# jyegerlehner/tensorflow-wavenet

Hardware: AMD Instinct MI355X
Metric: audio samples/sec (train, default wavenet_params.json) (higher is better)
Workload: dtype f32

## Files before the change

include/wavenet_hip.h:

```cpp
#ifndef WAVENET_HIP_H_
#define WAVENET_HIP_H_

#include <stdint.h>

#ifdef __cplusplus
extern "C" {
#endif

#define WN_OK 0
#define WN_ERR_BAD_SHAPE (-1)
#define WN_ERR_UNSUPPORTED (-2)
#define WN_ERR_MISALIGNED (-3)
#define WN_ERR_LAUNCH (-4)
#define WN_ERR_NULL (-5)

int wn_version(void);
const char* wn_error_string(int code);

int wn_mu_law_thresholds_host(int Q, float* thr_out);
int wn_mu_law_decode_table_host(int Q, float* lut_out);
int wn_mu_law_encode(const float* audio, int32_t* codes, long n,
                     const float* thr_dev, int Q, void* stream);
int wn_mu_law_decode(const int32_t* codes, float* audio, long n,
                     const float* lut_dev, int Q, void* stream);
// ... 55 lines not shown

int wn_layer_bwd2_slabs(int B, int T);
int wn_layer_bwd2_wimg_floats(void);
int wn_layer_bwd2_pack(const float* layer0, long layer_stride, float* wimg,
                       int L, void* stream);
int wn_layer_bwd2(const float* x, const float* z, const float* sg,
                  const float* dZ, const float* dxin, float* dx_out,
                  const float* wblock, const float* wimg, float* slabs,
                  float* tile_colsum, int B, int T, int dilation,
                  void* stream);

#define WN_STACK_VARIANT(rows, waves) (((rows) & 0x3f) | (((waves) & 0xf) << 8))
long wn_stack_flag_count(int B, int T, int L);
int wn_stack_tile_rows(int B, int T, int variant);
int wn_stack_wimg_floats(void);
int wn_stack_pack(const float* layer0, long layer_stride, float* wimg_fwd,
                  float* wimg_bwd, int L, void* stream);
int wn_stack_fwd(float* X, float* Z, float* SG, const float* wimg,
                 const float* bias, long bias_layer_stride,
                 int bias_clip_stride, const int* dilations, unsigned* flags,
                 unsigned* ctl, float* poison, int L, int B, int T, int save_sg,
                 int variant, void* stream);
int wn_stack_fwd_skip_ok(int B, int T, int S, int variant);
long wn_stack_skip_img_floats(int L);
int wn_stack_skip_pack(const float* skip_w, int L, float* img, void* stream);
int wn_stack_fwd_skip(float* X, float* Z, float* SG, const float* wimg,
                      const float* bias, long bias_layer_stride,
                      int bias_clip_stride, const int* dilations, unsigned* flags,
                      unsigned* ctl, float* poison, int L, int B, int T, int save_sg,
                      int variant, const float* skip_img, const float* skip_bsum,
                      float* h1, void* stream);
int wn_stack_fwd_lc(float* X, float* Z, float* SG, const float* wimg,
                    const float* bias, long bias_layer_stride,
                    int bias_clip_stride, const int* dilations, unsigned* flags,
                    unsigned* ctl, float* poison, int L, int B, int T, int save_sg,
                    int variant, const float* lc_add, long lc_row_stride,
                    void* stream);
int wn_stack_bwd_slabs(int B, int T, int variant);
int wn_stack_fwd_waves(int B, int T, int variant);
int wn_stack_bwd_waves(int B, int T, int variant, int* tiles_per_wave);
int wn_stack_bwd(const float* X, const float* Z, const float* SG,
                 const float* dZ, float* DX, long dx_layer_stride, float* Q,
                 const float* wimg, float* slabs,
                 long slab_layer_stride, float* tilesum, const int* dilations,
                 unsigned* flags, unsigned* ctl, float* poison, int L, int B,
                 int T, int variant, void* stream);
int wn_stack_bwd_lc(const float* X, const float* Z, const float* SG,
                    const float* dZ, float* DX, long dx_layer_stride, float* Q,
                    const float* wimg, float* slabs,
                    long slab_layer_stride, float* tilesum, const int* dilations,
                    unsigned* flags, unsigned* ctl, float* poison, int L, int B,
                    int T, int variant, float* lc_da, long lc_row_stride,
                    void* stream);

int wn_gemm_nn(const float* A, long lda, int a_planes, long a_plane_stride,
               const float* W, int ldw, const float* bias, const float* mask,
               long ld_mask, const float* addend, long ld_add, float* C,
               long ldc, int c_planes, long c_plane_stride, float* Cpre,
               long M, int N, int K, int relu, void* stream);

long wn_gemm_split_w_bytes(int K, int N);
int wn_gemm_nn_split(const float* A, long lda, int a_planes,
                     long a_plane_stride, const float* W, int ldw,
                     const float* bias, const float* mask, long ld_mask,
                     const float* addend, long ld_add, float* C, long ldc,
                     int c_planes, long c_plane_stride, float* Cpre, long M,
                     int N, int K, int relu, void* w_scratch, int nprod,
                     void* stream);
long wn_gemm_tn_slab_floats(int Mw, int Nw);
int wn_gemm_tn_tail_rows(int Mw, int Nw);
int wn_gemm_tn_splits(long rows, int Mw, int Nw, int kind);
int wn_gemm_tn_split(const float* A, long lda, int a_planes,
                     long a_plane_stride, const float* G, long ldg,
                     float* slabs, int splits, long rows, int Mw, int Nw,
                     int want_colsum, int nprod, void* stream);
int wn_gemm_tn(const float* A, long lda, int a_planes, long a_plane_stride,
               const int32_t* codes, int shift, int T, const float* G,
               long ldg, float* slabs, int splits, long rows, int Mw, int Nw,
               int want_colsum, void* stream);
int wn_reduce_slabs(const float* slabs, int num_slabs, long slab_stride,
                    int batch, long in_batch_stride, long offset, long n,
                    float* dst, long out_batch_stride, int replicate,
                    long rep_stride, void* stream);
int wn_reduce_slabs_mt(const float* slabs, int num_slabs, long slab_stride,
                       long n_main, float* dst_main, long n_tail, float* dst_tail,
                       int replicate, long rep_stride, int tail_rows, void* stream);
int wn_reduce_pair_slabs(const float* slabs, int num_slabs, int CB, int K,
                         int has_dense, int use_bias, float* layer_grad, int C,
                         long off_bias, int tap0, int Ktot, void* stream);
int wn_transpose(const float* in, int rows, int cols, long in_ld, float* out,
                 long out_ld, void* stream);

int wn_xent_partials(long rows);
int wn_xent(const float* logits, long ld, const int32_t* q, float* dlogits,
            float* loss_partials, int B, int T, int Q, int tf_quirk,
            void* stream);
int wn_xent_masked(const float* logits, long ld, const int32_t* q,
                   const int32_t* lengths, const float* inv_den,
                   float* dlogits, float* loss_partials, int B, int T, int Q,
                   int tf_quirk, void* stream);
int wn_xent_window(const float* logits, long ld, const int32_t* q,
                   const int32_t* starts, const int32_t* lengths,
                   const float* inv_den, float* dlogits, float* loss_partials,
                   int B, int T, int Q, int tf_quirk, void* stream);
long wn_xent_score_scratch_floats(long rows);
int wn_xent_score(const float* logits, long ld, const int32_t* q,
                  const int32_t* lengths, float* row_nll, double* clip_nll,
                  int32_t* clip_count, int32_t* clip_correct, float* scratch,
                  int B, int T, int Q, void* stream);
int wn_xent_score_window(const float* logits, long ld, const int32_t* q,
                         const int32_t* starts, const int32_t* lengths,
                         float* row_nll, double* clip_nll, int32_t* clip_count,
                         int32_t* clip_correct, float* scratch, int B, int T,
                         int Q, void* stream);
int wn_softmax64_row(const float* logits_row, int Q, float* proba,
                     void* stream);

int wn_adam(float* p, const float* g, float* m, float* v, long n, float lr_t,
            float beta1, float beta2, float eps, float grad_scale, float l2,
            const float* l2_mask, void* stream);
int wn_momentum(float* p, const float* g, float* acc, long n, float lr,
                float momentum, float grad_scale, float l2,
                const float* l2_mask, void* stream);
int wn_rmsprop(float* p, const float* g, float* ms, float* mom, long n,
               float lr, float decay, float momentum, float eps,
               float grad_scale, float l2, const float* l2_mask,
               void* stream);
int wn_grad_norm_partials_count(void);
int wn_grad_norm_partials(const float* g, long n, double* partials,
                          void* stream);
int wn_adam_clip(float* p, const float* g, float* m, float* v, long n,
                 float lr_t, float beta1, float beta2, float eps,
                 float grad_scale, float l2, const float* l2_mask,
                 const double* partials, int nparts, float clip_norm,
                 float* ema, float ema_decay, float* norm_out, void* stream);
int wn_momentum_clip(float* p, const float* g, float* acc, long n, float lr,
                     float momentum, float grad_scale, float l2,
                     const float* l2_mask, const double* partials, int nparts,
                     float clip_norm, float* ema, float ema_decay,
                     float* norm_out, void* stream);
int wn_rmsprop_clip(float* p, const float* g, float* ms, float* mom, long n,
                    float lr, float decay, float momentum, float eps,
                    float grad_scale, float l2, const float* l2_mask,
                    const double* partials, int nparts, float clip_norm,
                    float* ema, float ema_decay, float* norm_out,
                    void* stream);
int wn_l2_partials_count(void);
int wn_l2_partials(const float* p, long n, const float* mask, float* partials,
                   void* stream);

int wn_gc_bias(const float* layer0, long layer_stride, long off_bias,
               long off_gc, int G, const float* emb, int card,
               const int32_t* ids, float* out, int L, int B, int ch,
               void* stream);
int wn_colsum_clip_chunks(int T);
int wn_colsum_clip(const float* plane0, const float* plane1, int B, int T,
                   float* part, float* out, void* stream);
int wn_gc_grad(const float* layer0, long layer_stride, long off_gc, int G,
               const float* emb, int card, const int32_t* ids,
               const float* dsum, int L, int B, float* glayer0, float* gemb,
               float* scratch , int ch, void* stream);

int wn_causal_conv(const float* x, const float* w, float* y, int B, int T,
                   int Cin, int Cout, int K, int dilation, void* stream);
int wn_time_to_batch(const float* in, float* out, int B, int T, int C,
                     int dilation, void* stream);
int wn_batch_to_time(const float* in, float* out, int B_out, int U, int C,
                     int dilation, void* stream);

int wn_diag_mfma_peak(float* out, int blocks, int iters, void* stream);

int wn_axpy(float* y, const float* x, float a, const float* mask, long n,
            void* stream);
int wn_fill(float* p, long n, float value, void* stream);
int wn_sum_rows(const float* in, int rows, int n, float* out, void* stream);

long wn_fastgen_state_floats(const int32_t* dilations_host, int L);
int wn_fastgen_init(float* state, long state_floats, int32_t* cursors, int L,
                    void* stream);
int wn_fastgen_run(const float* params_causal, const float* layer0,
                   long layer_stride, const float* skip_w,
                   const float* skip_bsum, const float* post1_w,
                   const float* post1_b, const float* post2_w,
                   const float* post2_b, const float* gc_bias_fg,
                   const int32_t* dilations_dev, int L, int S, int Q,
                   float* state, int32_t* cursors, int32_t* samples_io,
                   int n_given, int n_steps, float temperature, uint64_t seed,
                   float* proba_out, int proba_every, int use_biases,
                   int push, void* stream);

long wn_fastgen_wide_coop_bytes(int L, int C, int S, int Q);
int wn_fastgen_run_wide(const float* params_causal, const float* layer0,
                        long layer_stride, const float* skip_w,
                        const float* skip_bsum, const float* post1_w,
                        const float* post1_b, const float* post2_w,
                        const float* post2_b, const float* gc_bias_fg,
                        const int32_t* dilations_dev, int L, int C, int S, int Q,
                        float* state, int32_t* cursors, int32_t* samples_io,
                        int n_given, int n_steps, float temperature,
                        uint64_t seed, float* proba_out, int proba_every,
                        int use_biases, int push, void* coop, void* stream);

int wn_fastgen_step(const float* params_causal, const float* layer0,
                    long layer_stride, const float* skip_w,
                    const float* skip_bsum, const float* post1_w,
                    const float* post1_b, const float* post2_w,
                    const float* post2_b, const float* gc_bias_fg,
                    const int32_t* dilations_dev, int L, int S, int Q,
                    float* state, int32_t* cursors, int32_t* samples_io,
                    const int32_t* ctl, float* proba_out, int use_biases,
                    const float* cw_img, float* pre, float* z_all, float* h1,
                    float* h2, float* logits, void* stream);
int wn_fastgen_finish(int Q, int32_t* cursors, int32_t* samples_io,
                      const int32_t* ctl, float* proba_out, const float* logits,
                      void* stream);

int wn_fastgen_persist_workgroups(int L, int S, int Q);
int wn_fastgen_persist_role(int block, int total, int nseg);
long wn_fastgen_persist_ll_words(int L, int S, int Q);
int wn_fastgen_persist(const float* params_causal, const float* layer0,
                       long layer_stride, const float* skip_w,
                       const float* skip_bsum, const float* post1_w,
                       const float* post1_b, const float* post2_w,
                       const float* post2_b, const float* gc_bias_fg,
                       const int32_t* dilations_dev, int L, int S, int Q,
                       float* state, int32_t* cursors, int32_t* samples_io,
                       const int32_t* ctl, float* proba_out, int use_biases,
                       const float* cw_img, float* pre, float* z_all, float* h1,
                       float* h2, float* logits, unsigned* sync,
                       unsigned long long* ll, int n_steps, void* stream);
int wn_fastgen_pre(const float* layer0, long layer_stride,
                   const float* gc_bias_fg, const int32_t* dilations_dev,
                   int L, const float* state, const int32_t* cursors,
                   float* pre, void* stream);
int wn_fastgen_pack(const float* layer0, long layer_stride, float* img, int L,
                    void* stream);

int wn_fastgen_batch_rows(int B);
long wn_fastgen_batch_state_floats(const int32_t* dilations_host, int L, int B);
int wn_fastgen_batch_init(float* state, long state_floats, int32_t* cursors,
                          int32_t* prev, int B, void* stream);
int wn_fastgen_batch_pre(const float* layer0, long layer_stride,
                         const float* gc_bias_fg, int bias_stream_stride,
                         const int32_t* dilations_dev, int L, int B,
                         const float* state, const int32_t* cursors, float* pre,
                         void* stream);
int wn_fastgen_batch_step(const float* params_causal, const float* layer0,
                          long layer_stride, const float* skip_w,
                          const float* skip_bsum, const float* post1_w,
                          const float* post1_b, const float* post2_w,
                          const float* post2_b, const float* gc_bias_fg,
                          int bias_stream_stride, const int32_t* dilations_dev,
                          int L, int S, int Q, int B, float* state,
                          int32_t* cursors, int32_t* prev, int32_t* samples_io,
                          const int32_t* ctl, const uint64_t* seeds,
                          float* proba_out, int use_biases, float* pre,
                          float* z_all, float* h1, float* h2, float* logits,
                          void* stream);
// ... 203 lines not shown
```

tensorflow-wavenet_amd/csrc/wn_gemm.hip:

```cpp
#include "wn_common.h"
#include <cstdlib>
#include <cstddef>
#include <cstring>

struct GemmNN {
  const float* A;
  long lda;
  long a_plane_stride;
  int a_planes;
  const float* W;
  int ldw;
  const float* bias;
  const float* mask;
  long ld_mask;
  const float* addend;
  long ld_add;
  float* C;
  long ldc;
  long c_plane_stride;
  int c_planes;
  float* Cpre;
  long M;
  int N, K;
  int relu;
  int tiles_n;
  int nwg;
  int tiles_m;
  int tile_rows;
};

typedef const __attribute__((address_space(1))) void* gptr_t;
typedef __attribute__((address_space(3))) void* lptr_t;

#define NN_TM 128
#define NN_TN 128
#define NN_KC 32
#ifndef NN3_PF
#define NN3_PF 2
#endif

__device__ __forceinline__ int xcd_remap(int bid, int nwg) {
  const int q = nwg >> 3, r = nwg & 7, xcd = bid & 7, idx = bid >> 3;
  const int base = xcd < r ? xcd * (q + 1) : r * (q + 1) + (xcd - r) * q;
  return base + idx;
}

#define EP_LD 68
#ifndef EP_ST_AUX
#define EP_ST_AUX 2
#endif
#ifndef EP_LD_AUX
#define EP_LD_AUX 2
#endif
typedef unsigned ep_u32x4 __attribute__((ext_vector_type(4)));
__device__ __forceinline__ __amdgpu_buffer_rsrc_t ep_rsrc(const float* base) {
  return __builtin_amdgcn_make_buffer_rsrc((void*)base, 0, 0x7fffffff, 0x00020000);
}
__device__ __forceinline__ void gemm_epilogue(const GemmNN& g, f32x16 (&acc)[2][2],
                                              float* lds, long m0, int n0,
                                              int wm, int wn, int wave, int lane,
                                              long m_end = -1) {
  if (m_end < 0) m_end = g.M;
  const int j = lane & 31, h = lane >> 5;
  float* tile = lds + wave * (32 * EP_LD);
  const int rr = lane >> 4, cc = (lane & 15) * 4;
  const int nw = n0 + wn * 64;
  const bool ncol = nw + cc < g.N;
  f32x4 bias4 = {0.f, 0.f, 0.f, 0.f};
  if (g.bias && ncol) bias4 = *reinterpret_cast<const f32x4*>(g.bias + nw + cc);
  const int vC = g.c_planes ? (int)(((long)(cc >> 5) * g.c_plane_stride + rr * 32 + (cc & 31)) * 4)
                            : (int)((rr * g.ldc + cc) * 4);
  const int sC = g.c_planes ? 4 * 32 * 4 : (int)(4 * g.ldc * 4);
  const int vP = (int)((rr * g.ldc + cc) * 4);
  const int sP = (int)(4 * g.ldc * 4);
  const int vM = (int)((rr * g.ld_mask + cc) * 4), sM = (int)(4 * g.ld_mask * 4);
  const bool addp = g.addend && g.c_planes && g.ld_add == 0;
  const int vA = addp ? vC : (int)((rr * g.ld_add + cc) * 4);
  const int sA = addp ? sC : (int)(4 * g.ld_add * 4);
#pragma unroll
  for (int fm = 0; fm < 2; ++fm) {
    __builtin_amdgcn_wave_barrier();
#pragma unroll
    for (int fn = 0; fn < 2; ++fn)
// ... 1087 lines not shown

  const int prow = lane >> 5, pcol = (lane & 31) * 4;
  int am = m0 + pcol;
  am = am < g.Mw ? am : g.Mw - 4;
  int gn = n0 + pcol;
  gn = gn < g.Nw ? gn : g.Nw - 4;
  auto stage = [&](int c, int st) {
    float* base = smem + st * STAGE;
    const long r0 = r_begin + (long)c * KR;
#pragma unroll
    for (int q = 0; q < 2; ++q) {
      const int p = wave + 4 * q;
      const long row = r0 + 2 * p + prow;
      const float* src = g.a_planes
                             ? g.A + (long)(am >> 5) * g.a_plane_stride + row * 32 + (am & 31)
                             : g.A + row * g.lda + am;
      __builtin_amdgcn_global_load_lds((gptr_t)src, (lptr_t)(base + p * 256), 16, 0, 0);
      __builtin_amdgcn_global_load_lds((gptr_t)(g.G + row * g.ldg + gn),
                                       (lptr_t)(base + KR * TT + p * 256), 16, 0, 0);
    }
  };

  f32x16 acc[2][2];
#pragma unroll
  for (int a = 0; a < 2; ++a)
#pragma unroll
    for (int b = 0; b < 2; ++b) acc[a][b] = frag_zero();
  float cs[2] = {0.f, 0.f};

  if (nchunks > 0) stage(0, 0);
  for (int c = 0; c < nchunks; ++c) {
    const int st = c & 1;
    asm volatile("s_waitcnt vmcnt(0)\n\ts_barrier" ::: "memory");
    if (c + 1 < nchunks) stage(c + 1, st ^ 1);
    const float* al = smem + st * STAGE + 8 * h * TT + wm * 64 + i;
    const float* gl = smem + st * STAGE + KR * TT + 8 * h * TT + wn * 64 + i;
    Split3 as[2], gs[2];
#pragma unroll
    for (int f = 0; f < 2; ++f) {
      float v[8];
#pragma unroll
      for (int e = 0; e < 8; ++e) v[e] = al[e * TT + f * 32];
      as[f] = split3(v);
    }
#pragma unroll
    for (int f = 0; f < 2; ++f) {
      float v[8];
#pragma unroll
      for (int e = 0; e < 8; ++e) {
        v[e] = gl[e * TT + f * 32];
        cs[f] += v[e];
      }
      gs[f] = split3(v);
    }
#pragma unroll
    for (int a = 0; a < 2; ++a)
#pragma unroll
      for (int b = 0; b < 2; ++b) mma_split<NPROD>(acc[a][b], as[a], gs[b]);
  }

  float* slab = g.slabs + (long)split * g.slab_stride;
#pragma unroll
  for (int a = 0; a < 2; ++a)
#pragma unroll
    for (int b = 0; b < 2; ++b) {
      const int n = n0 + wn * 64 + b * 32 + i;
      if (n >= g.Nw) continue;
#pragma unroll
      for (int rr = 0; rr < 16; ++rr) {
        const int m = m0 + wm * 64 + a * 32 + 8 * (rr >> 2) + 4 * h + (rr & 3);
        if (m < g.Mw) slab[(long)m * g.Nw + n] = acc[a][b][rr];
      }
    }
  if (g.want_colsum && tm == 0 && wm == 0) {
#pragma unroll
    for (int b = 0; b < 2; ++b) {
      const float v = cs[b] + __shfl_xor(cs[b], 32);
      const int n = n0 + wn * 64 + b * 32 + i;
      if (h == 0 && n < g.Nw) slab[(long)g.Mw * g.Nw + n] = v;
    }
  }
}

__global__ void reduce_slabs_kernel(const float* __restrict__ slabs,
                                    int num_slabs, long slab_stride,
                                    long in_batch_stride, long offset, long n,
                                    float* __restrict__ dst,
                                    long out_batch_stride, int replicate,
                                    long rep_stride) {
  const long e = (long)blockIdx.x * blockDim.x + threadIdx.x;
  if (e >= n) return;
  const int b = blockIdx.y;
  const float* p = slabs + (long)b * in_batch_stride + offset + e;
  float s0 = 0.f, s1 = 0.f, s2 = 0.f, s3 = 0.f;
  int s = 0;
  for (; s + 3 < num_slabs; s += 4) {
    s0 += p[(long)s * slab_stride];
    s1 += p[(long)(s + 1) * slab_stride];
    s2 += p[(long)(s + 2) * slab_stride];
    s3 += p[(long)(s + 3) * slab_stride];
  }
  for (; s < num_slabs; ++s) s0 += p[(long)s * slab_stride];
  const float v = (s0 + s1) + (s2 + s3);
  for (int r = 0; r < replicate; ++r)
    dst[(long)b * out_batch_stride + (long)r * rep_stride + e] = v;
}

template <int PARTS>
__global__ void reduce_slabs4_kernel(const float* __restrict__ slabs,
                                     int num_slabs, long slab_stride,
                                     long in_batch_stride, long offset, long n4,
                                     float* __restrict__ dst,
                                     long out_batch_stride, int replicate,
                                     long rep_stride) {
  __shared__ f32x4 part[PARTS > 1 ? PARTS : 1][64];
  const int col = threadIdx.x & 63, pt = threadIdx.x >> 6;
  const long e = (long)blockIdx.x * 64 + col;
  const int b = blockIdx.y;
  const int per = (num_slabs + PARTS - 1) / PARTS;
  const int s0 = pt * per, s1 = min(num_slabs, s0 + per);
  f32x4 acc[8];
#pragma unroll
  for (int k = 0; k < 8; ++k) acc[k] = f32x4{0.f, 0.f, 0.f, 0.f};
  if (e < n4) {
    const f32x4* p = reinterpret_cast<const f32x4*>(slabs + (long)b * in_batch_stride + offset) + e;
    const long st = slab_stride / 4;
    int s = s0;
    for (; s + 7 < s1; s += 8) {
      f32x4 v[8];
#pragma unroll
      for (int k = 0; k < 8; ++k) v[k] = p[(long)(s + k) * st];
#pragma unroll
      for (int k = 0; k < 8; ++k) acc[k] += v[k];
    }
#pragma unroll
    for (int k = 0; k < 7; ++k)
      if (s + k < s1) acc[k] += p[(long)(s + k) * st];
  }
  f32x4 v = ((acc[0] + acc[1]) + (acc[2] + acc[3])) + ((acc[4] + acc[5]) + (acc[6] + acc[7]));
  if (PARTS > 1) {
    part[pt][col] = v;
    __syncthreads();
    if (pt != 0) return;
    if (PARTS == 4) v = (part[0][col] + part[1][col]) + (part[2][col] + part[3][col]);
    else v = part[0][col] + part[1][col];
  }
  if (e >= n4) return;
  for (int r = 0; r < replicate; ++r)
    *reinterpret_cast<f32x4*>(dst + (long)b * out_batch_stride + (long)r * rep_stride + 4 * e) = v;
}

#ifndef RMT_PARTS
#define RMT_PARTS 4
#endif
__global__ __launch_bounds__(64 * RMT_PARTS) void reduce_slabs_mt_kernel(
    const float* __restrict__ slabs, int num_slabs, long slab_stride, long n_main4,
    float* __restrict__ dst_main, long n_tail4, float* __restrict__ dst_tail,
    int replicate, long rep_stride, int tail_rows) {
  __shared__ f32x4 part[RMT_PARTS][64];
  const int col = threadIdx.x & 63, pt = threadIdx.x >> 6;
  const long e = (long)blockIdx.x * 64 + col;
  const long n4 = n_main4 + n_tail4;
  const int per = (num_slabs + RMT_PARTS - 1) / RMT_PARTS;
  const int s0 = min(num_slabs, pt * per), s1 = min(num_slabs, s0 + per);
  f32x4 acc[8];
#pragma unroll
  for (int k = 0; k < 8; ++k) acc[k] = f32x4{0.f, 0.f, 0.f, 0.f};
  if (e < n4) {
    const f32x4* p = reinterpret_cast<const f32x4*>(slabs) + e;
    const long st = slab_stride / 4;
    int s = s0;
    for (; s + 7 < s1; s += 8) {
      f32x4 v[8];
#pragma unroll
      for (int k = 0; k < 8; ++k) v[k] = p[(long)(s + k) * st];
#pragma unroll
      for (int k = 0; k < 8; ++k) acc[k] += v[k];
    }
#pragma unroll
    for (int k = 0; k < 7; ++k)
      if (s + k < s1) acc[k] += p[(long)(s + k) * st];
    if (e >= n_main4 && tail_rows > 1) {
      const int nv = (s1 - s0) * (tail_rows - 1);
      int v = 0;
      for (; v + 7 < nv; v += 8) {
        f32x4 w[8];
#pragma unroll
        for (int k = 0; k < 8; ++k) {
          const int q = s0 + (v + k) / (tail_rows - 1), t = 1 + (v + k) % (tail_rows - 1);
          w[k] = p[(long)q * st + (long)t * n_tail4];
        }
#pragma unroll
        for (int k = 0; k < 8; ++k) acc[k] += w[k];
      }
      for (; v < nv; ++v) {
        const int q = s0 + v / (tail_rows - 1), t = 1 + v % (tail_rows - 1);
        acc[v & 7] += p[(long)q * st + (long)t * n_tail4];
      }
    }
  }
  part[pt][col] = ((acc[0] + acc[1]) + (acc[2] + acc[3])) + ((acc[4] + acc[5]) + (acc[6] + acc[7]));
  __syncthreads();
  if (pt != 0 || e >= n4) return;
  f32x4 v = f32x4{0.f, 0.f, 0.f, 0.f};
#pragma unroll
  for (int q = 0; q < RMT_PARTS; q += 4)
    v += (part[q][col] + part[q + 1][col]) + (part[q + 2][col] + part[q + 3][col]);
  if (e < n_main4) {
    reinterpret_cast<f32x4*>(dst_main)[e] = v;
  } else {
    for (int r = 0; r < replicate; ++r)
      *reinterpret_cast<f32x4*>(dst_tail + (long)r * rep_stride + 4 * (e - n_main4)) = v;
  }
}

#define RPS_PARTS 16
__global__ __launch_bounds__(64 * RPS_PARTS) void reduce_pair_slabs_kernel(
    const float* __restrict__ slabs, int num_slabs, int CB, int K, int has_dense,
    int use_bias, float* __restrict__ g, int C, long off_bias, int tap0, int Ktot) {
  __shared__ f32x4 part[RPS_PARTS][64];
  const int WF = (2 * K + 1) * 1024, n4 = (WF + 96) / 4;
  const int col = threadIdx.x & 63, pt = threadIdx.x >> 6;
  const int e4 = blockIdx.x * 64 + col;
  const int pair = blockIdx.y, a = pair / CB, b = pair - a * CB;
  const int per = (num_slabs + RPS_PARTS - 1) / RPS_PARTS;
  const int s0 = min(num_slabs, pt * per), s1 = min(num_slabs, s0 + per);
  f32x4 acc[8];
#pragma unroll
  for (int k = 0; k < 8; ++k) acc[k] = f32x4{0.f, 0.f, 0.f, 0.f};
  if (e4 < n4) {
    const f32x4* p = reinterpret_cast<const f32x4*>(
                         slabs + (size_t)pair * num_slabs * (WF + 96)) + e4;
    const long st = (WF + 96) / 4;
    int s = s0;
    for (; s + 7 < s1; s += 8) {
      f32x4 v[8];
#pragma unroll
      for (int k = 0; k < 8; ++k) v[k] = p[(long)(s + k) * st];
#pragma unroll
      for (int k = 0; k < 8; ++k) acc[k] += v[k];
    }
#pragma unroll
    for (int k = 0; k < 7; ++k)
      if (s + k < s1) acc[k] += p[(long)(s + k) * st];
  }
  part[pt][col] = ((acc[0] + acc[1]) + (acc[2] + acc[3])) + ((acc[4] + acc[5]) + (acc[6] + acc[7]));
  __syncthreads();
  if (pt != 0 || e4 >= n4) return;
  f32x4 v = f32x4{0.f, 0.f, 0.f, 0.f};
#pragma unroll
  for (int q = 0; q < RPS_PARTS; q += 4)
    v += (part[q][col] + part[q + 1][col]) + (part[q + 2][col] + part[q + 3][col]);
  const int e = 4 * e4;
  if (e < WF) {
    const int m = e >> 10, r = (e >> 5) & 31, c = e & 31;
    if (m == 2 * K && !has_dense) return;
    const int md = m < K ? tap0 + m : m < 2 * K ? Ktot + tap0 + (m - K) : 2 * Ktot;
    *reinterpret_cast<f32x4*>(g + ((size_t)md * C + a * 32 + r) * C + b * 32 + c) = v;
  } else if (a == 0 && use_bias) {
    const int q = (e - WF) >> 5, c = (e - WF) & 31;
    if (q == 2 && !has_dense) return;
    *reinterpret_cast<f32x4*>(g + off_bias + (size_t)q * C + b * 32 + c) = v;
  }
}

__global__ void transpose_pad_kernel(const float* __restrict__ in, int rows,
                                     int cols, long in_ld,
                                     float* __restrict__ out, long out_ld) {
  __shared__ float tile[32][33];
  const int bx = blockIdx.x * 32, by = blockIdx.y * 32;
  const int tx = threadIdx.x & 31, ty = threadIdx.x >> 5;
  for (int k = ty; k < 32; k += 8) {
    const int r = by + k, c = bx + tx;
    tile[k][tx] = (r < rows && c < cols) ? in[(long)r * in_ld + c] : 0.f;
  }
  __syncthreads();
  for (int k = ty; k < 32; k += 8) {
    const int c = bx + k, r = by + tx;
    if (c < cols && r < rows) out[(long)c * out_ld + r] = tile[tx][k];
  }
}

template <int MODE>
__global__ __launch_bounds__(256) void mfma_peak_kernel(float* out, int iters) {
  __shared__ float lds[4096];
  for (int k = threadIdx.x; k < 4096; k += 256) lds[k] = 1.0f + k * 1e-4f;
  __syncthreads();
  f32x16 a0 = frag_zero(), a1 = frag_zero(), a2 = frag_zero(), a3 = frag_zero();
  float x = 1.0f + threadIdx.x * 1e-3f, y = 0.5f - threadIdx.x * 1e-3f;
  const float* lp = lds + (threadIdx.x & 63);
  for (int it = 0; it < iters; ++it) {
#pragma unroll
    for (int u = 0; u < 8; ++u) {
      if (MODE == 1) {
        x = lp[(u * 128 + it) & 4095 & ~63];
        y = lp[((u * 128 + 64 + it) & 4095) & ~63];
      }
      a0 = __builtin_amdgcn_mfma_f32_32x32x2f32(x, y, a0, 0, 0, 0);
      a1 = __builtin_amdgcn_mfma_f32_32x32x2f32(y, x, a1, 0, 0, 0);
      a2 = __builtin_amdgcn_mfma_f32_32x32x2f32(x, x, a2, 0, 0, 0);
      a3 = __builtin_amdgcn_mfma_f32_32x32x2f32(y, y, a3, 0, 0, 0);
    }
  }
  float s = 0.f;
#pragma unroll
  for (int r = 0; r < 16; ++r) s += a0[r] + a1[r] + a2[r] + a3[r];
  out[blockIdx.x * 256 + threadIdx.x] = s;
}

extern "C" {

int wn_diag_mfma_peak(float* out, int blocks, int iters, void* stream) {
  if (!out) return WN_ERR_NULL;
  if (blocks <= 0 || iters == 0) return WN_ERR_BAD_SHAPE;
  if (iters > 0)
    hipLaunchKernelGGL(mfma_peak_kernel<0>, dim3(blocks), dim3(256), 0,
                       (hipStream_t)stream, out, iters);
  else
    hipLaunchKernelGGL(mfma_peak_kernel<1>, dim3(blocks), dim3(256), 0,
                       (hipStream_t)stream, out, -iters);
  return wn_check_launch();
}

static int gemm_nn_describe(GemmNN& g, const float* A, long lda, int a_planes,
               long a_plane_stride, const float* W, int ldw, const float* bias,
               const float* mask, long ld_mask, const float* addend, long ld_add,
               float* C, long ldc, int c_planes, long c_plane_stride, float* Cpre,
               long M, int N, int K, int relu) {
  if (!A || !W || !C) return WN_ERR_NULL;
  if (M <= 0 || N <= 0 || K <= 0) return WN_ERR_BAD_SHAPE;
  if ((N & 3) || (K & 3) || (ldw & 3)) return WN_ERR_UNSUPPORTED;
  if (a_planes) {
    if (K != a_planes * 32) return WN_ERR_BAD_SHAPE;
  } else if (lda & 3) {
    return WN_ERR_UNSUPPORTED;
  }
  if (c_planes) {
    if (N != c_planes * 32) return WN_ERR_BAD_SHAPE;
  } else if (ldc & 3) {
    return WN_ERR_UNSUPPORTED;
  }
  if ((mask && (ld_mask & 3)) || (addend && (ld_add & 3)))
    return WN_ERR_UNSUPPORTED;
  if (addend && ld_add == 0 && !c_planes) return WN_ERR_BAD_SHAPE;
  if (c_planes && c_plane_stride * 4 >= (1L << 31)) return WN_ERR_UNSUPPORTED;
  const void* ptrs[] = {A, W, bias, mask, addend, C, Cpre};
  for (const void* p : ptrs)
    if (p && !wn_aligned16(p)) return WN_ERR_MISALIGNED;
  g.A = A; g.lda = lda; g.a_plane_stride = a_plane_stride; g.a_planes = a_planes;
  g.W = W; g.ldw = ldw; g.bias = bias; g.mask = mask; g.ld_mask = ld_mask;
  g.addend = addend; g.ld_add = ld_add; g.C = C; g.ldc = ldc;
  g.c_plane_stride = c_plane_stride; g.c_planes = c_planes; g.Cpre = Cpre;
  g.M = M; g.N = N; g.K = K; g.relu = relu;
  long tiles_m = (M + NN_TM - 1) / NN_TM;
  g.tiles_n = (N + NN_TN - 1) / NN_TN;
  g.tile_rows = NN_TM;
  const long nwg = tiles_m * g.tiles_n;
  if (nwg > 0x7fffffffL) return WN_ERR_BAD_SHAPE;
  g.nwg = (int)nwg;
  g.tiles_m = (int)tiles_m;
  return WN_OK;
}

// ... 135 lines not shown
  g.tiles_m = (Mw + 127) / 128;
  g.tiles_n = (Nw + 127) / 128;
  dim3 grid(g.tiles_m * g.tiles_n, splits), block(256);
  hipStream_t s = (hipStream_t)stream;
  if (nprod == 3) hipLaunchKernelGGL(gemm_tn_split_kernel<3>, grid, block, 0, s, g);
  else if (nprod == 9) hipLaunchKernelGGL(gemm_tn_split_kernel<9>, grid, block, 0, s, g);
  else hipLaunchKernelGGL(gemm_tn_split_kernel<6>, grid, block, 0, s, g);
  return wn_check_launch();
}

int wn_gemm_tn(const float* A, long lda, int a_planes, long a_plane_stride,
               const int32_t* codes, int shift, int T, const float* G,
               long ldg, float* slabs, int splits, long rows, int Mw, int Nw,
               int want_colsum, void* stream) {
  if (!G || !slabs) return WN_ERR_NULL;
  if (!A && !codes) return WN_ERR_NULL;
  if (rows <= 0 || Mw <= 0 || Nw <= 0 || splits <= 0) return WN_ERR_BAD_SHAPE;
  if (a_planes && Mw != a_planes * 32) return WN_ERR_BAD_SHAPE;
  if (codes && T <= 0) return WN_ERR_BAD_SHAPE;
  GemmTN g;
  g.A = A; g.lda = lda; g.a_plane_stride = a_plane_stride; g.a_planes = a_planes;
  g.codes = codes; g.shift = shift; g.T = T > 0 ? T : 1; g.G = G; g.ldg = ldg;
  g.slabs = slabs; g.slab_stride = wn_gemm_tn_slab_floats(Mw, Nw);
  g.rows = rows;
  long rps = (rows + splits - 1) / splits;
  rps = (rps + 95) / 96 * 96;
  g.rows_per_split = rps;
  g.Mw = Mw; g.Nw = Nw; g.want_colsum = want_colsum;
  hipStream_t s = (hipStream_t)stream;
  if (!codes && (lda % 4 == 0) && (ldg % 4 == 0) && wn_aligned16(A) &&
      wn_aligned16(G)) {
    int mf2 = 0, nf2 = 0;
    tn_wg_tile(Mw, Nw, &mf2, &nf2);
    if (mf2 && nf2) {
      g.tiles_m = Mw / (mf2 * 32);
      g.tiles_n = Nw / (4 * nf2 * 32);
      dim3 grid2(g.tiles_m * g.tiles_n, splits), block2(256);
      const long rps = (rows + splits - 1) / splits + 96;
      const long a_bytes = (a_planes ? 5 * a_plane_stride + rps * 32 : rps * lda) * 4;
      const bool dma = a_bytes < (1L << 31) && rps * ldg * 4 < (1L << 31);
#define LAUNCH2(mf, nf)                                                          \
  do {                                                                           \
    if (dma) hipLaunchKernelGGL((gemm_tn3_kernel<mf, nf>), grid2, block2, 0, s, g); \
    else hipLaunchKernelGGL((gemm_tn2_kernel<mf, nf>), grid2, block2, 0, s, g);  \
  } while (0)
      if (mf2 == 5 && nf2 == 2) LAUNCH2(5, 2);
      else if (mf2 == 5) LAUNCH2(5, 1);
      else if (nf2 == 2) LAUNCH2(4, 2);
      else LAUNCH2(4, 1);
#undef LAUNCH2
      return wn_check_launch();
    }
  }
  if (want_colsum == 2) return WN_ERR_UNSUPPORTED;
  const int m32 = (Mw + 31) / 32, n32 = (Nw + 31) / 32;
  int NF = (n32 % 2 == 0) ? 2 : 1;
  int MF;
  if (codes) { NF = 1; MF = (m32 % 2 == 0) ? 2 : 1; }
  else if (m32 % 5 == 0) MF = 5;
  else if (m32 % 4 == 0) MF = 4;
  else if (m32 % 2 == 0) MF = 2;
  else MF = 1;
  g.tiles_m = (m32 + MF - 1) / MF;
  g.tiles_n = (n32 + NF - 1) / NF;
  const int wtiles = g.tiles_m * g.tiles_n;
  dim3 grid((wtiles + 3) / 4, splits), block(256);
#define LAUNCH(mf, nf) \
  hipLaunchKernelGGL((gemm_tn_kernel<mf, nf>), grid, block, 0, s, g)
  if (NF == 2) {
    if (MF == 5) LAUNCH(5, 2);
    else if (MF == 4) LAUNCH(4, 2);
    else if (MF == 2) LAUNCH(2, 2);
    else LAUNCH(1, 2);
  } else {
    if (MF == 5) LAUNCH(5, 1);
    else if (MF == 4) LAUNCH(4, 1);
    else if (MF == 2) LAUNCH(2, 1);
    else LAUNCH(1, 1);
  }
#undef LAUNCH
  return wn_check_launch();
}

__global__ __launch_bounds__(64) void reduce_slabs_wave_kernel(
    const float* __restrict__ slabs, int num_slabs, long slab_stride,
    long in_batch_stride, long offset, float* __restrict__ dst,
    long out_batch_stride, int replicate, long rep_stride) {
  const long e = blockIdx.x;
  const int b = blockIdx.y;
  const float* p = slabs + (long)b * in_batch_stride + offset + e;
  float v = 0.f;
  for (int s = threadIdx.x; s < num_slabs; s += 64) v += p[(long)s * slab_stride];
#pragma unroll
  for (int o = 32; o >= 1; o >>= 1) v += __shfl_xor(v, o);
  if (threadIdx.x == 0)
    for (int r = 0; r < replicate; ++r)
      dst[(long)b * out_batch_stride + (long)r * rep_stride + e] = v;
}

int wn_reduce_slabs(const float* slabs, int num_slabs, long slab_stride,
                    int batch, long in_batch_stride, long offset, long n,
                    float* dst, long out_batch_stride, int replicate,
                    long rep_stride, void* stream) {
  if (!slabs || !dst) return WN_ERR_NULL;
  if (num_slabs <= 0 || n <= 0 || batch <= 0 || replicate <= 0)
    return WN_ERR_BAD_SHAPE;
  if (n <= 4 && num_slabs >= 256) {
    hipLaunchKernelGGL(reduce_slabs_wave_kernel, dim3((unsigned)n, batch),
                       dim3(64), 0, (hipStream_t)stream, slabs, num_slabs,
                       slab_stride, in_batch_stride, offset, dst,
                       out_batch_stride, replicate, rep_stride);
    return wn_check_launch();
  }
  if (((n | offset | slab_stride | in_batch_stride | out_batch_stride | rep_stride) & 3) == 0 &&
      wn_aligned16(slabs) && wn_aligned16(dst)) {
    const long n4 = n / 4;
    dim3 grid4((unsigned)((n4 + 63) / 64), batch);
    const bool split = num_slabs >= 32 && (long)grid4.x * batch <= 4096;
    if (split)
      hipLaunchKernelGGL(reduce_slabs4_kernel<4>, grid4, dim3(256), 0, (hipStream_t)stream,
                         slabs, num_slabs, slab_stride, in_batch_stride, offset, n4,
                         dst, out_batch_stride, replicate, rep_stride);
    else
      hipLaunchKernelGGL(reduce_slabs4_kernel<1>, grid4, dim3(64), 0, (hipStream_t)stream,
                         slabs, num_slabs, slab_stride, in_batch_stride, offset, n4,
                         dst, out_batch_stride, replicate, rep_stride);
    return wn_check_launch();
  }
  dim3 grid((unsigned)((n + 255) / 256), batch), block(256);
  hipLaunchKernelGGL(reduce_slabs_kernel, grid, block, 0, (hipStream_t)stream,
                     slabs, num_slabs, slab_stride, in_batch_stride, offset, n,
                     dst, out_batch_stride, replicate, rep_stride);
  return wn_check_launch();
}

int wn_reduce_slabs_mt(const float* slabs, int num_slabs, long slab_stride,
                       long n_main, float* dst_main, long n_tail, float* dst_tail,
                       int replicate, long rep_stride, int tail_rows, void* stream) {
  if (!slabs || !dst_main || (n_tail > 0 && !dst_tail)) return WN_ERR_NULL;
  if (num_slabs <= 0 || n_main <= 0 || n_tail < 0 || replicate < 1 || tail_rows < 1 ||
      slab_stride < n_main + (long)tail_rows * n_tail)
    return WN_ERR_BAD_SHAPE;
  if (((n_main | n_tail | slab_stride | rep_stride) & 3) != 0) return WN_ERR_UNSUPPORTED;
  if (!wn_aligned16(slabs) || !wn_aligned16(dst_main) || (dst_tail && !wn_aligned16(dst_tail)))
    return WN_ERR_MISALIGNED;
  const long n4 = (n_main + n_tail) / 4;
  hipLaunchKernelGGL(reduce_slabs_mt_kernel, dim3((unsigned)((n4 + 63) / 64)), dim3(64 * RMT_PARTS), 0,
                     (hipStream_t)stream, slabs, num_slabs, slab_stride, n_main / 4, dst_main,
                     n_tail / 4, dst_tail, replicate, rep_stride, tail_rows);
  return wn_check_launch();
}

int wn_reduce_pair_slabs(const float* slabs, int num_slabs, int CB, int K,
                         int has_dense, int use_bias, float* layer_grad, int C,
                         long off_bias, int tap0, int Ktot, void* stream) {
  if (!slabs || !layer_grad) return WN_ERR_NULL;
  if (num_slabs <= 0 || CB <= 0 || K < 1 || C != CB * 32 || off_bias < 0 || (off_bias & 3) ||
      tap0 < 0 || Ktot < tap0 + K)
    return WN_ERR_BAD_SHAPE;
  if (!wn_aligned16(slabs) || !wn_aligned16(layer_grad)) return WN_ERR_MISALIGNED;
  const int n4 = ((2 * K + 1) * 1024 + 96) / 4;
  hipLaunchKernelGGL(reduce_pair_slabs_kernel, dim3((n4 + 63) / 64, CB * CB), dim3(64 * RPS_PARTS), 0,
                     (hipStream_t)stream, slabs, num_slabs, CB, K, has_dense, use_bias,
                     layer_grad, C, off_bias, tap0, Ktot);
  return wn_check_launch();
}

int wn_transpose(const float* in, int rows, int cols, long in_ld, float* out,
                 long out_ld, void* stream) {
  if (!in || !out) return WN_ERR_NULL;
  if (rows <= 0 || cols <= 0) return WN_ERR_BAD_SHAPE;
  dim3 grid((cols + 31) / 32, (rows + 31) / 32), block(256);
  hipLaunchKernelGGL(transpose_pad_kernel, grid, block, 0, (hipStream_t)stream,
                     in, rows, cols, in_ld, out, out_ld);
  return wn_check_launch();
}

}
```

tensorflow-wavenet_amd/csrc/wn_misc.hip:

```cpp
#include "wn_common.h"
#include <stdlib.h>
#include <cmath>

#pragma clang fp contract(off)
static inline int mu_chain_host(float x, int Q) {
  const float mu = (float)(Q - 1);
  const float ax = std::fabs(x);
  const float arg = 1.0f + mu * ax;
  const float num = (float)std::log((double)arg);
  const float den = (float)std::log((double)(1.0f + mu));
  const float mag = num / den;
  const float sgn = (x > 0.f) ? 1.f : ((x < 0.f) ? -1.f : 0.f);
  float v = sgn * mag;
  v = v + 1.0f;
  v = v / 2.0f;
  v = v * mu;
  v = v + 0.5f;
  return (int)v;
}

static inline uint32_t f2key(float f) {
  uint32_t u;
  __builtin_memcpy(&u, &f, 4);
  return (u & 0x80000000u) ? ~u : (u | 0x80000000u);
}
static inline float key2f(uint32_t k) {
  uint32_t u = (k & 0x80000000u) ? (k & 0x7FFFFFFFu) : ~k;
  float f;
  __builtin_memcpy(&f, &u, 4);
  return f;
}

__device__ __forceinline__ int mu_chain_dev(float x, int Q) {
  const float mu = (float)(Q - 1);
  const float arg = __fadd_rn(1.0f, __fmul_rn(mu, fabsf(x)));
  const float num = (float)log((double)arg);
  const float den = (float)log((double)__fadd_rn(1.0f, mu));
  const float mag = __fdiv_rn(num, den);
  const float sgn = (x > 0.f) ? 1.f : ((x < 0.f) ? -1.f : 0.f);
  float v = __fmul_rn(sgn, mag);
  v = __fadd_rn(v, 1.0f);
  v = __fdiv_rn(v, 2.0f);
  v = __fmul_rn(v, mu);
  v = __fadd_rn(v, 0.5f);
  return (int)v;
}

__global__ void mu_law_encode_kernel(const float* __restrict__ audio,
                                     int32_t* __restrict__ codes, long n,
                                     const float* __restrict__ thr, int Q) {
  extern __shared__ float sthr[];
  for (int i = threadIdx.x; i < Q - 1; i += blockDim.x) sthr[i] = thr[i];
  __syncthreads();
  for (long idx = (long)blockIdx.x * blockDim.x + threadIdx.x; idx < n;
       idx += (long)gridDim.x * blockDim.x) {
    const float x = audio[idx];
    int code;
    if (x >= -1.f && x <= 1.f) {
      int lo = 0, hi = Q - 1;
      while (lo < hi) {
        const int mid = (lo + hi) >> 1;
        if (sthr[mid] <= x) lo = mid + 1; else hi = mid;
      }
      code = lo;
    } else {
      code = mu_chain_dev(x, Q);
    }
    codes[idx] = code;
  }
}

__device__ __forceinline__ float mu_decode_dev(int code, int Q) {
  const float mu = (float)(Q - 1);
  const float s = __fsub_rn(__fmul_rn(2.0f, __fdiv_rn((float)code, mu)), 1.0f);
  const float p = (float)pow((double)__fadd_rn(1.0f, mu), (double)fabsf(s));
  const float mag = __fmul_rn(__fdiv_rn(1.0f, mu), __fsub_rn(p, 1.0f));
  const float sgn = (s > 0.f) ? 1.f : ((s < 0.f) ? -1.f : 0.f);
  return __fmul_rn(sgn, mag);
}

__global__ void mu_law_decode_kernel(const int32_t* __restrict__ codes,
                                     float* __restrict__ audio, long n,
                                     const float* __restrict__ lut, int Q) {
  for (long idx = (long)blockIdx.x * blockDim.x + threadIdx.x; idx < n;
       idx += (long)gridDim.x * blockDim.x) {
    const int c = codes[idx];
    audio[idx] = (c >= 0 && c < Q) ? lut[c] : mu_decode_dev(c, Q);
  }
}

__global__ void causal_gather_kernel(const int32_t* __restrict__ q,
                                     const float* __restrict__ Wc,
                                     float* __restrict__ x0, long rows, int T,
                                     int Q, int K, int ldw) {
  const long idx = (long)blockIdx.x * blockDim.x + threadIdx.x;
  const long row = idx >> 3;
  const int c4 = (idx & 7) * 4;
  if (row >= rows) return;
  const int t = (int)(row % T);
  f32x4 v = {0.f, 0.f, 0.f, 0.f};
  const int extra = (K - 1) / 2;
  for (int k = 0; k < K; ++k) {
    const int s = (K - 1 - k) + extra;
    if (t < s) continue;
    const int code = q[row - s];
    if (code >= 0 && code < Q)
      v += *reinterpret_cast<const f32x4*>(Wc + ((long)k * Q + code) * ldw + c4);
  }
  *reinterpret_cast<f32x4*>(x0 + row * 32 + c4) = v;
}

__global__ void scalar_causal_fwd_kernel(const float* __restrict__ audio,
                                         const float* __restrict__ W,
                                         float* __restrict__ x0, long rows,
                                         int T, int K0, int ldw) {
  const long idx = (long)blockIdx.x * blockDim.x + threadIdx.x;
  const long row = idx >> 3;
  const int c4 = (idx & 7) * 4;
  if (row >= rows) return;
  const int t = (int)(row % T);
  f32x4 v = {0.f, 0.f, 0.f, 0.f};
  const int extra = (K0 - 1) / 2;
  for (int k = 0; k < K0; ++k) {
    const int s = (K0 - 1 - k) + extra;
    if (t - s < 0) continue;
    const float a = audio[row - s];
    const f32x4 w = *reinterpret_cast<const f32x4*>(W + (long)k * ldw + c4);
    v += a * w;
  }
  *reinterpret_cast<f32x4*>(x0 + row * 32 + c4) = v;
}

__global__ __launch_bounds__(1024) void scalar_causal_wgrad_kernel(
    const float* __restrict__ audio, const float* __restrict__ dx0,
    float* __restrict__ slabs, long rows, long rows_per_split, int T, int K0) {
  const int c = threadIdx.x & 31;
  const long r0 = (long)blockIdx.x * rows_per_split;
  long r1 = r0 + rows_per_split;
  if (r1 > rows) r1 = rows;
  for (int k = threadIdx.x >> 5; k < K0; k += 32) {
    const int s = (K0 - 1 - k) + (K0 - 1) / 2;
    float acc = 0.f;
    int t = (int)(r0 % T);
    for (long r = r0; r < r1; ++r) {
      if (t >= s) acc = fmaf(audio[r - s], dx0[r * 32 + c], acc);
      if (++t == T) t = 0;
    }
    slabs[(long)blockIdx.x * K0 * 32 + k * 32 + c] = acc;
  }
}

__global__ void gc_bias_kernel(const float* __restrict__ layer0, long layer_stride,
                               long off_bias, long off_gc, int G,
                               const float* __restrict__ emb, int card,
                               const int32_t* __restrict__ ids,
                               float* __restrict__ out, int B, int ch) {
  const int l = blockIdx.x, b = blockIdx.y;
  const float* blk = layer0 + (long)l * layer_stride;
  for (int c = threadIdx.x; c < 2 * ch; c += blockDim.x) {
    float v = blk[off_bias + c];
    if (emb) {
      const int id = ids[b];
      if (id >= 0 && id < card) {
        const float* w = blk + off_gc + (c >= ch ? (long)G * ch : 0) + (c % ch);
        const float* e = emb + (long)id * G;
        for (int g = 0; g < G; ++g) v += e[g] * w[(long)g * ch];
      }
    }
    out[((long)l * B + b) * 2 * ch + c] = v;
  }
}

__global__ __launch_bounds__(256) void colsum_clip_kernel(
    const float* __restrict__ P0, const float* __restrict__ P1, int T,
    int rows_per_chunk, float* __restrict__ part) {
  __shared__ float red[8][64];
  const int b = blockIdx.y, chunk = blockIdx.x;
  const int c = threadIdx.x & 31, w = threadIdx.x >> 5;
  const int t0 = chunk * rows_per_chunk;
  const int t1 = min(T, t0 + rows_per_chunk);
  const float* p0 = P0 + (long)b * T * 32;
  const float* p1 = P1 + (long)b * T * 32;
  float s0 = 0.f, s1 = 0.f;
  for (int t = t0 + w; t < t1; t += 8) {
    s0 += p0[(long)t * 32 + c];
    s1 += p1[(long)t * 32 + c];
  }
  red[w][c] = s0;
  red[w][32 + c] = s1;
  __syncthreads();
  if (threadIdx.x < 64) {
    float v = 0.f;
// ... 43 lines not shown
                                   float* __restrict__ gemb) {
  extern __shared__ float tmp[];
  const int tid = threadIdx.x;
  for (int e = tid; e < card * G; e += blockDim.x) gemb[e] = 0.f;
  for (int e = tid; e < B * G; e += blockDim.x) {
    float s = 0.f;
    for (int l = 0; l < L; ++l) s += part[(long)l * B * G + e];
    tmp[e] = s;
  }
  __syncthreads();
  for (int gi = tid; gi < G; gi += blockDim.x) {
    for (int b = 0; b < B; ++b) {
      const int id = ids[b];
      if (id < 0 || id >= card) continue;
      gemb[(long)id * G + gi] += tmp[b * G + gi];
    }
  }
}

__global__ void causal_conv_kernel(const float* __restrict__ x,
                                   const float* __restrict__ w,
                                   float* __restrict__ y, int B, int T, int Cin,
                                   int Cout, int K, int d) {
  const long idx = (long)blockIdx.x * blockDim.x + threadIdx.x;
  const long total = (long)B * T * Cout;
  if (idx >= total) return;
  const int co = (int)(idx % Cout);
  const long bt = idx / Cout;
  const int t = (int)(bt % T);
  const long b = bt / T;
  float acc = 0.f;
  for (int k = 0; k < K; ++k) {
    const long shift = (long)(K - 1 - k + (K - 1) / 2) * d;
    if (t - shift < 0) continue;
    const float* xr = x + ((b * T) + (t - shift)) * Cin;
    const float* wk = w + (long)k * Cin * Cout + co;
    for (int ci = 0; ci < Cin; ++ci) acc += xr[ci] * wk[(long)ci * Cout];
  }
  y[idx] = acc;
}

__global__ void time_to_batch_kernel(const float* __restrict__ in,
                                     float* __restrict__ out, int B, int T,
                                     int C, int d, int U) {
  const long idx = (long)blockIdx.x * blockDim.x + threadIdx.x;
  const long total = (long)B * d * U * C;
  if (idx >= total) return;
  const int c = (int)(idx % C);
  long r = idx / C;
  const int u = (int)(r % U);
  r /= U;
  const int b = (int)(r % B), p = (int)(r / B);
  const long t = (long)u * d + p;
  out[idx] = t < T ? in[((long)b * T + t) * C + c] : 0.f;
}

__global__ void batch_to_time_kernel(const float* __restrict__ in,
                                     float* __restrict__ out, int B, int U,
                                     int C, int d) {
  const long idx = (long)blockIdx.x * blockDim.x + threadIdx.x;
  const long total = (long)B * d * U * C;
  if (idx >= total) return;
  const int c = (int)(idx % C);
  long r = idx / C;
  const int tt = (int)(r % ((long)U * d));
  const int b = (int)(r / ((long)U * d));
  const int u = tt / d, p = tt % d;
  out[idx] = in[(((long)p * B + b) * U + u) * C + c];
}

__global__ void axpy_kernel(float* __restrict__ y, const float* __restrict__ x,
                            float a, const float* __restrict__ mask, long n) {
  for (long i = (long)blockIdx.x * blockDim.x + threadIdx.x; i < n;
       i += (long)gridDim.x * blockDim.x)
    y[i] += a * x[i] * (mask ? mask[i] : 1.f);
}

__global__ void fill_kernel(float* __restrict__ p, long n, float v) {
  for (long i = (long)blockIdx.x * blockDim.x + threadIdx.x; i < n;
       i += (long)gridDim.x * blockDim.x)
    p[i] = v;
}

__global__ void sum_rows_kernel(const float* __restrict__ in, int rows, int n,
                                float* __restrict__ out) {
  const int c = blockIdx.x * blockDim.x + threadIdx.x;
  if (c >= n) return;
  float s = 0.f;
  int r = 0;
  for (; r + 16 <= rows; r += 16) {
    float v[16];
#pragma unroll
    for (int u = 0; u < 16; ++u) v[u] = in[(long)(r + u) * n + c];
#pragma unroll
    for (int u = 0; u < 16; ++u) s += v[u];
  }
  for (; r < rows; ++r) s += in[(long)r * n + c];
  out[c] = s;
}

extern "C" {

int wn_reduce_slabs(const float* slabs, int num_slabs, long slab_stride,
                    int batch, long in_batch_stride, long offset, long n,
                    float* dst, long out_batch_stride, int replicate,
                    long rep_stride, void* stream);

int wn_version(void) { return 100; }

const char* wn_error_string(int code) {
  switch (code) {
    case WN_OK: return "ok";
    case WN_ERR_BAD_SHAPE: return "bad shape";
    case WN_ERR_UNSUPPORTED: return "unsupported configuration";
    case WN_ERR_MISALIGNED: return "pointer or leading dimension not 16-byte aligned";
    case WN_ERR_LAUNCH: return "kernel launch failed";
    case WN_ERR_NULL: return "null pointer";
    default: return "unknown error";
  }
}

int wn_mu_law_thresholds_host(int Q, float* thr_out) {
  if (!thr_out) return WN_ERR_NULL;
  if (Q < 2) return WN_ERR_BAD_SHAPE;
  const uint32_t lo0 = f2key(-1.0f), hi0 = f2key(1.0f);
  for (int k = 1; k < Q; ++k) {
    uint32_t lo = lo0, hi = hi0;
    if (mu_chain_host(key2f(lo), Q) >= k) { thr_out[k - 1] = key2f(lo); continue; }
    while (hi - lo > 1) {
      const uint32_t mid = lo + (hi - lo) / 2;
      if (mu_chain_host(key2f(mid), Q) >= k) hi = mid; else lo = mid;
    }
    thr_out[k - 1] = key2f(hi);
  }
  return WN_OK;
}

int wn_mu_law_decode_table_host(int Q, float* lut_out) {
  if (!lut_out) return WN_ERR_NULL;
  if (Q < 2) return WN_ERR_BAD_SHAPE;
  const float mu = (float)(Q - 1);
  for (int c = 0; c < Q; ++c) {
    float s = (float)c / mu;
    s = 2.0f * s;
    s = s - 1.0f;
    const float p = (float)std::pow((double)(1.0f + mu), (double)std::fabs(s));
    float mag = 1.0f / mu;
    const float pm1 = p - 1.0f;
    mag = mag * pm1;
    const float sgn = (s > 0.f) ? 1.f : ((s < 0.f) ? -1.f : 0.f);
    lut_out[c] = sgn * mag;
  }
  return WN_OK;
}

int wn_mu_law_encode(const float* audio, int32_t* codes, long n,
                     const float* thr_dev, int Q, void* stream) {
  if (!audio || !codes || !thr_dev) return WN_ERR_NULL;
  if (n <= 0 || Q < 2 || Q > 8192) return WN_ERR_BAD_SHAPE;
  hipLaunchKernelGGL(mu_law_encode_kernel, dim3(grid1d(n, 256)), dim3(256),
                     (Q - 1) * sizeof(float), (hipStream_t)stream, audio, codes,
                     n, thr_dev, Q);
  return wn_check_launch();
}

int wn_mu_law_decode(const int32_t* codes, float* audio, long n,
                     const float* lut_dev, int Q, void* stream) {
  if (!audio || !codes || !lut_dev) return WN_ERR_NULL;
  if (n <= 0 || Q < 2) return WN_ERR_BAD_SHAPE;
  hipLaunchKernelGGL(mu_law_decode_kernel, dim3(grid1d(n, 256)), dim3(256), 0,
                     (hipStream_t)stream, codes, audio, n, lut_dev, Q);
  return wn_check_launch();
}

int wn_causal_gather(const int32_t* q, const float* Wc, float* x0, int B,
                     int T, int Q, int K, int ldw, void* stream) {
  if (!q || !Wc || !x0) return WN_ERR_NULL;
  if (B <= 0 || T <= 0 || Q <= 0 || K <= 0 || ldw < 32 || (ldw & 3))
    return WN_ERR_BAD_SHAPE;
  if (!wn_aligned16(Wc) || !wn_aligned16(x0)) return WN_ERR_MISALIGNED;
  const long rows = (long)B * T;
// ... 180 lines not shown
                     plane0, plane1, T, rpc, part);
  return wn_reduce_slabs(part, chunks, 64, B, (long)chunks * 64, 0, 64, out, 64,
                         1, 0, stream);
}

int wn_gc_grad(const float* layer0, long layer_stride, long off_gc, int G,
               const float* emb, int card, const int32_t* ids,
               const float* dsum, int L, int B, float* glayer0, float* gemb,
               float* scratch, int ch, void* stream) {
  if (!layer0 || !emb || !ids || !dsum || !glayer0 || !gemb || !scratch)
    return WN_ERR_NULL;
  if (L <= 0 || B <= 0 || G <= 0 || card <= 0 || ch < 32) return WN_ERR_BAD_SHAPE;
  if ((size_t)B * G * sizeof(float) > 48 * 1024) return WN_ERR_UNSUPPORTED;
  hipStream_t s = (hipStream_t)stream;
  hipLaunchKernelGGL(gc_grad_kernel, dim3(2 * L), dim3(256), 0, s, layer0,
                     layer_stride, off_gc, G, emb, card, ids, dsum, L, B,
                     glayer0, scratch, ch);
  hipLaunchKernelGGL(gc_grad_emb_kernel, dim3(1), dim3(256),
                     (size_t)B * G * sizeof(float), s, scratch, L, B, G, card,
                     ids, gemb);
  return wn_check_launch();
}

int wn_causal_conv(const float* x, const float* w, float* y, int B, int T,
                   int Cin, int Cout, int K, int dilation, void* stream) {
  if (!x || !w || !y) return WN_ERR_NULL;
  if (B <= 0 || T <= 0 || Cin <= 0 || Cout <= 0 || K <= 0 || dilation <= 0)
    return WN_ERR_BAD_SHAPE;
  const long total = (long)B * T * Cout;
  hipLaunchKernelGGL(causal_conv_kernel, dim3((unsigned)((total + 255) / 256)),
                     dim3(256), 0, (hipStream_t)stream, x, w, y, B, T, Cin,
                     Cout, K, dilation);
  return wn_check_launch();
}

int wn_time_to_batch(const float* in, float* out, int B, int T, int C,
                     int dilation, void* stream) {
  if (!in || !out) return WN_ERR_NULL;
  if (B <= 0 || T <= 0 || C <= 0 || dilation <= 0) return WN_ERR_BAD_SHAPE;
  const int U = (T + dilation - 1) / dilation;
  const long total = (long)B * dilation * U * C;
  hipLaunchKernelGGL(time_to_batch_kernel, dim3((unsigned)((total + 255) / 256)),
                     dim3(256), 0, (hipStream_t)stream, in, out, B, T, C,
                     dilation, U);
  return wn_check_launch();
}

int wn_batch_to_time(const float* in, float* out, int B_out, int U, int C,
                     int dilation, void* stream) {
  if (!in || !out) return WN_ERR_NULL;
  if (B_out <= 0 || U <= 0 || C <= 0 || dilation <= 0) return WN_ERR_BAD_SHAPE;
  const long total = (long)B_out * dilation * U * C;
  hipLaunchKernelGGL(batch_to_time_kernel, dim3((unsigned)((total + 255) / 256)),
                     dim3(256), 0, (hipStream_t)stream, in, out, B_out, U, C,
                     dilation);
  return wn_check_launch();
}

int wn_axpy(float* y, const float* x, float a, const float* mask, long n,
            void* stream) {
  if (!y || !x) return WN_ERR_NULL;
  if (n <= 0) return WN_ERR_BAD_SHAPE;
  hipLaunchKernelGGL(axpy_kernel, dim3(grid1d(n, 256)), dim3(256), 0,
                     (hipStream_t)stream, y, x, a, mask, n);
  return wn_check_launch();
}

int wn_fill(float* p, long n, float value, void* stream) {
  if (!p) return WN_ERR_NULL;
  if (n <= 0) return WN_ERR_BAD_SHAPE;
  hipLaunchKernelGGL(fill_kernel, dim3(grid1d(n, 256)), dim3(256), 0,
                     (hipStream_t)stream, p, n, value);
  return wn_check_launch();
}

int wn_sum_rows(const float* in, int rows, int n, float* out, void* stream) {
  if (!in || !out) return WN_ERR_NULL;
  if (rows <= 0 || n <= 0) return WN_ERR_BAD_SHAPE;
  hipLaunchKernelGGL(sum_rows_kernel, dim3((n + 255) / 256), dim3(256), 0,
                     (hipStream_t)stream, in, rows, n, out);
  return wn_check_launch();
}

}
```

tensorflow-wavenet_amd/csrc/wn_stack.hip:

```cpp
#include "wn_common.h"

#define WN_WAIT_VM0() asm volatile("s_waitcnt vmcnt(0)" ::: "memory")
#define WN_WAIT_LGKM0() asm volatile("s_waitcnt lgkmcnt(0)" ::: "memory")

#define STACK_MAXL 256
#define SF_LD 36
#define SF_MT (32 * SF_LD)
#define SF_OFF_BD (5 * SF_MT)
#define STACK_WBUF 5888

struct StackFwd {
  float* X;
  float* Z;
  float* SG;
  const float* wimg;
  const float* bias;
  long bias_layer_stride;
  int bias_clip_stride;
  const int* dil;
  unsigned* flags;
  unsigned* ctl;
  float* poison;
  int L, B, T;
  long plane;
  const float* skimg;
  const float* sk_bsum;
  float* sk_out;
#ifdef STACK_STAMPS
  unsigned long long* dbg;
#endif
};

#define SK_S 512
#define SK_NT 8
#define SK_WAVE (SK_NT * 2 * 256)
#define SK_AHEAD 3
#define SK_ZB 4

typedef unsigned u32x4 __attribute__((ext_vector_type(4)));

__device__ __forceinline__ RowRegs rows_load_dev(const float* tile0, int lane,
                                                 int lo, int hi) {
  RowRegs R;
  __amdgpu_buffer_rsrc_t rs = __builtin_amdgcn_make_buffer_rsrc(
      (void*)tile0, 0, 0x7fffffff, 0x00020000);
  const int vo = ((lane >> 3) * 32 + (lane & 7) * 4) * 4;
#pragma unroll
  for (int c = 0; c < 4; ++c) {
    const int r = 8 * c + (lane >> 3);
    f32x4 v = {0.f, 0.f, 0.f, 0.f};
    if (r >= lo && r < hi)
      v = __builtin_bit_cast(
          f32x4, __builtin_amdgcn_raw_buffer_load_b128(rs, vo + c * 1024, 0, 16));
    R.v[c] = v;
  }
  return R;
}

template <int AUX>
__device__ __forceinline__ void rows_store_aux(float* tile0, int lane, int hi,
                                               const RowRegs& R) {
  __amdgpu_buffer_rsrc_t rs = __builtin_amdgcn_make_buffer_rsrc(
      (void*)tile0, 0, 0x7fffffff, 0x00020000);
  const int vo = ((lane >> 3) * 32 + (lane & 7) * 4) * 4;
#pragma unroll
  for (int c = 0; c < 4; ++c) {
    const int r = 8 * c + (lane >> 3);
    if (r < hi)
      __builtin_amdgcn_raw_buffer_store_b128(__builtin_bit_cast(u32x4, R.v[c]),
                                             rs, vo + c * 1024, 0, AUX);
  }
}
__device__ __forceinline__ void rows_store_dev(float* tile0, int lane, int hi,
                                               const RowRegs& R) {
  rows_store_aux<16>(tile0, lane, hi, R);
}

__device__ __forceinline__ void wait_flags(const unsigned* fl, int idx,
                                           unsigned epoch, unsigned* ctl,
                                           float* poison, bool& dead, int lane) {
  if (dead) return;
  unsigned spins = 0;
  unsigned long long t_start = 0;
  for (;;) {
    bool pending = false;
    if (idx >= 0)
      pending = __hip_atomic_load(fl + idx, __ATOMIC_RELAXED,
                                  __HIP_MEMORY_SCOPE_AGENT) != epoch;
    if (__builtin_amdgcn_ballot_w64(pending) == 0) break;
    if ((++spins & 63u) == 0) {
      const unsigned long long now = __builtin_amdgcn_s_memrealtime();
      if (t_start == 0) t_start = now;
      if (now - t_start > 200000000ull) {
        if (lane == 0) {
          __hip_atomic_store(ctl + 3, 1u, __ATOMIC_RELAXED, __HIP_MEMORY_SCOPE_AGENT);
          if (poison) *poison = __builtin_nanf("");
        }
        dead = true;
        break;
      }
    }
    __builtin_amdgcn_s_sleep(1);
  }
  asm volatile("" ::: "memory");
}

__device__ __forceinline__ void mma32t_chain(f32x16& acc, const f32x16& frag,
                                             const float* wt_lane, f32x4& pre,
                                             const float* wt_next) {
  f32x4 nxt = pre;
#pragma unroll
  for (int q = 0; q < 4; ++q) {
    const f32x4 a4 = nxt;
    nxt = *reinterpret_cast<const f32x4*>(q < 3 ? wt_lane + 8 * (q + 1) : wt_next);
    __builtin_amdgcn_sched_barrier(0);
#pragma unroll
    for (int e = 0; e < 4; ++e)
      acc = __builtin_amdgcn_mfma_f32_32x32x2f32(a4[e], frag[4 * q + e], acc, 0, 0, 0);
    __builtin_amdgcn_sched_barrier(0);
  }
  pre = nxt;
}

__global__ void stack_pack_kernel(const float* __restrict__ layer0,
                                  long layer_stride, float* __restrict__ img_f,
                                  float* __restrict__ img_b) {
  const bool bwd = blockIdx.y == 1;
  float* img = bwd ? img_b : img_f;
  if (!img) return;
  const float* blk = layer0 + (long)blockIdx.x * layer_stride;
  float* out = img + (size_t)blockIdx.x * STACK_WBUF;
  for (int i = threadIdx.x; i < STACK_WBUF; i += blockDim.x) out[i] = 0.f;
  __syncthreads();
  for (int i = threadIdx.x; i < LAYER_W_FLOATS; i += blockDim.x) {
    const int m = i >> 10, cin = (i >> 5) & 31, cout = i & 31;
    out[bwd ? m * 1024 + cin * 32 + ((((cout >> 2) ^ ((cin >> 1) & 7)) << 2) | (cout & 3))
            : m * SF_MT + cout * SF_LD + cin] = blk[i];
  }
  if (!bwd && threadIdx.x < 32)
    out[SF_OFF_BD + threadIdx.x] = blk[LAYER_OFF_BD + threadIdx.x];
}

__device__ __forceinline__ void wait_lds(const int* p, bool& dead, unsigned* ctl,
                                         float* poison, int lane) {
  unsigned spins = 0;
  while (!dead && __hip_atomic_load(p, __ATOMIC_RELAXED, __HIP_MEMORY_SCOPE_WORKGROUP) == 0) {
    __builtin_amdgcn_s_sleep(1);
    if (++spins > (1u << 24)) {
      dead = true;
      if (lane == 0) {
        __hip_atomic_store(ctl + 3, 1u, __ATOMIC_RELAXED, __HIP_MEMORY_SCOPE_AGENT);
        if (poison) *poison = __builtin_nanf("");
      }
    }
  }
  asm volatile("" ::: "memory");
}

__global__ void stack_skip_pack_kernel(const float* __restrict__ skip_w, float* __restrict__ img) {
  const int l = blockIdx.x >> 2, j = blockIdx.x & 3;
  float* out = img + (size_t)blockIdx.x * SK_WAVE;
  for (int i = threadIdx.x; i < SK_WAVE; i += blockDim.x) {
    const int e = i & 3, lane = (i >> 2) & 63, half = (i >> 8) & 1, nt = i >> 9;
    const int jr = lane & 15, g = lane >> 4;
    out[i] = skip_w[((size_t)l * 32 + 16 * half + 4 * g + e) * SK_S + 128 * j + 16 * nt + jr];
  }
}

struct StackLc {
  float* p;
  long row_stride;
};
__device__ __forceinline__ StackLc stack_lc_arg(StackLc lc) { return lc; }

template <int SAVE, int WAVES, typename... Lc>
__global__ __launch_bounds__(WAVES * 64) void stack_fwd_kernel(StackFwd a, Lc... lc_) {
  constexpr bool LC = sizeof...(Lc) > 0;
  __shared__ __attribute__((aligned(1024))) float wl[2 * STACK_WBUF];
  __shared__ __attribute__((aligned(16))) float tiles[WAVES * 1024];
  __shared__ int s_group;
  __shared__ int s_done[STACK_MAXL], s_ready[STACK_MAXL];
  const int tid = threadIdx.x;
  const int lane = tid & 63;
  const int wave = __builtin_amdgcn_readfirstlane(tid >> 6);
  const int j = lane & 31, h = lane >> 5;
  const int T = a.T, L = a.L;
  const int tiles_per_clip = (T + 31) >> 5;
  const int ntiles = tiles_per_clip * a.B;
  const int ngroups = (ntiles + WAVES - 1) / WAVES;
  const unsigned epoch =
      __hip_atomic_load(a.ctl + 2, __ATOMIC_RELAXED, __HIP_MEMORY_SCOPE_AGENT);
  float* ta = tiles + wave * 1024;
  bool dead = false;
#ifdef STACK_STAMPS
#define SSTAMP(l, i)                                                         \
  if (lane == 0)                                                             \
    a.dbg[(((size_t)blockIdx.x * 16 + wave) * L + (l)) * 12 + (i)] =         \
        __builtin_amdgcn_s_memtime()
  unsigned long long* cal = a.dbg + (size_t)gridDim.x * 16 * L * 12 + (size_t)blockIdx.x * 4;
  if (tid == 0) { cal[0] = __builtin_amdgcn_s_memrealtime(); cal[1] = __builtin_amdgcn_s_memtime(); }
#else
#define SSTAMP(l, i)
#endif

  auto issue_weights = [&](int l, int p0, int step) {
    const float* wb = a.wimg + (size_t)l * STACK_WBUF;
    float* dst = wl + (l & 1) * STACK_WBUF;
    for (int p = p0; p < STACK_WBUF / 256; p += step)
      __builtin_amdgcn_global_load_lds((wn_gptr_t)(wb + p * 256 + lane * 4),
                                       (wn_lptr_t)(dst + p * 256), 16, 0, 0);
  };

  for (;;) {
    if (tid == 0) s_group = (int)atomicAdd(a.ctl, 1u);
    __syncthreads();
    const int g = __builtin_amdgcn_readfirstlane(s_group);
    __syncthreads();
    if (g >= ngroups) break;
    const int tile = g * WAVES + wave;
    const int nactive = min(WAVES, ntiles - g * WAVES);
    const bool any = tile < ntiles;
    const int b = any ? tile / tiles_per_clip : 0;
    const int tt = any ? tile - b * tiles_per_clip : 0;
// ... 1894 lines not shown
```

tensorflow-wavenet_amd/wavenet/_lib.py:

```python
import ctypes
import os

_HERE = os.path.dirname(os.path.abspath(__file__))
LIB_PATH = os.environ.get('WN_LIB_PATH') or os.path.join(
    os.path.dirname(_HERE), 'libwavenet_hip.so')

c_int, c_long, c_float = ctypes.c_int, ctypes.c_long, ctypes.c_float
c_void_p, c_u64 = ctypes.c_void_p, ctypes.c_uint64
P = c_void_p

SIGNATURES = {
    'wn_version': (c_int, []),
    'wn_error_string': (ctypes.c_char_p, [c_int]),
    'wn_mu_law_thresholds_host': (c_int, [c_int, P]),
    'wn_mu_law_decode_table_host': (c_int, [c_int, P]),
    'wn_mu_law_encode': (c_int, [P, P, c_long, P, c_int, P]),
    'wn_mu_law_decode': (c_int, [P, P, c_long, P, c_int, P]),
    'wn_causal_gather': (c_int, [P, P, P, c_int, c_int, c_int, c_int, c_int,
                                 P]),
    'wn_scalar_causal_fwd': (c_int, [P, P, c_int, P, c_int, c_int, c_int, P]),
    'wn_scalar_causal_wgrad': (c_int, [P, P, P, c_int, c_int, c_int, c_int,
                                       P]),
    'wn_causal_wgrad_slabs': (c_int, [c_long]),
    'wn_causal_wgrad': (c_int, [P, P, P, c_int, c_int, c_int, c_int, P]),
    'wn_layer_fwd': (c_int, [P, P, P, P, P, P, P, c_int, c_int, c_int, c_int,
                             c_int, c_int, P]),
    'wn_stack_flag_count': (c_long, [c_int, c_int, c_int]),
    'wn_stack_wimg_floats': (c_int, []),
    'wn_stack_tile_rows': (c_int, [c_int, c_int, c_int]),
    'wn_stack_pack': (c_int, [P, c_long, P, P, c_int, P]),
    'wn_stack_fwd': (c_int, [P, P, P, P, P, c_long, c_int, P, P, P, P,
                             c_int, c_int, c_int, c_int, c_int, P]),
    'wn_stack_fwd_skip': (c_int, [P, P, P, P, P, c_long, c_int, P, P, P, P,
                                  c_int, c_int, c_int, c_int, c_int, P, P, P, P]),
    'wn_stack_fwd_skip_ok': (c_int, [c_int, c_int, c_int, c_int]),
    'wn_stack_skip_img_floats': (c_long, [c_int]),
    'wn_stack_skip_pack': (c_int, [P, c_int, P, P]),
    'wn_stack_fwd_lc': (c_int, [P, P, P, P, P, c_long, c_int, P, P, P, P,
                                c_int, c_int, c_int, c_int, c_int, P, c_long,
                                P]),
    'wn_stack_bwd_slabs': (c_int, [c_int, c_int, c_int]),
    'wn_stack_fwd_waves': (c_int, [c_int, c_int, c_int]),
    'wn_stack_bwd_waves': (c_int, [c_int, c_int, c_int, P]),
    'wn_stack_bwd': (c_int, [P, P, P, P, P, c_long, P, P, P, c_long, P, P, P,
                             P, P, c_int, c_int, c_int, c_int, P]),
    'wn_stack_bwd_lc': (c_int, [P, P, P, P, P, c_long, P, P, P, c_long, P, P,
                                P, P, P, c_int, c_int, c_int, c_int, P, c_long,
                                P]),
    'wn_layer_wgrad_slab_floats': (c_int, []),
    'wn_dense_planes': (c_int, [P, c_long, P, P, P, c_long, P, c_long, c_long, c_int,
                                P]),
    'wn_dense_planes_gate': (c_int, [P, c_long, P, P, c_long, P, P, c_long, P, P,
                                     c_long, c_long, c_int, P]),
    'wn_layer_fwd_k': (c_int, [P, P, P, P, P, P, P, c_int, c_int, c_int, c_int,
                               c_int, c_int, c_int, P]),
    'wn_layer_bwd_k': (c_int, [P, P, P, P, P, P, P, P, P, P, P, c_int, c_int,
                               c_int, c_int, c_int, c_int, c_int, c_long, P]),
    'wn_layer_wgrad_k': (c_int, [P, P, P, P, P, P, c_int, c_int, c_int, c_int,
                                 c_int, c_int, c_int, c_int, c_long, P]),
    'wn_layer_fwd_blk': (c_int, [P, c_long, c_int, P, P, P, P, P, c_int, P, P,
                                 c_int, c_int, c_int, c_int, c_int, c_int,
                                 c_int, P, P, c_long, c_int, c_int, c_int,
                                 c_long, P]),
    'wn_layer_bwd_blk': (c_int, [P, P, c_long, c_int, P, P, P, P, c_int,
                                 c_long, c_int, c_int, c_int, c_int, c_int,
                                 c_int, c_int, c_long, P]),
    'wn_layer_bwd2_slabs': (c_int, [c_int, c_int]),
    'wn_layer_bwd2_wimg_floats': (c_int, []),
    'wn_layer_bwd2_pack': (c_int, [P, c_long, P, c_int, P]),
    'wn_layer_bwd2': (c_int, [P, P, P, P, P, P, P, P, P, P, c_int, c_int,
                              c_int, P]),
    'wn_gemm_nn': (c_int, [P, c_long, c_int, c_long, P, c_int, P, P, c_long,
                           P, c_long, P, c_long, c_int, c_long, P, c_long,
                           c_int, c_int, c_int, P]),
    'wn_gemm_split_w_bytes': (c_long, [c_int, c_int]),
    'wn_gemm_nn_split': (c_int, [P, c_long, c_int, c_long, P, c_int, P, P,
                                 c_long, P, c_long, P, c_long, c_int, c_long,
                                 P, c_long, c_int, c_int, c_int, P, c_int, P]),
    'wn_gemm_tn_tail_rows': (c_int, [c_int, c_int]),
    'wn_gemm_tn_slab_floats': (c_long, [c_int, c_int]),
    'wn_gemm_tn_splits': (c_int, [c_long, c_int, c_int, c_int]),
    'wn_gemm_tn_split': (c_int, [P, c_long, c_int, c_long, P, c_long, P, c_int,
                                 c_long, c_int, c_int, c_int, c_int, P]),
    'wn_gemm_tn': (c_int, [P, c_long, c_int, c_long, P, c_int, c_int, P,
                           c_long, P, c_int, c_long, c_int, c_int, c_int, P]),
    'wn_reduce_slabs': (c_int, [P, c_int, c_long, c_int, c_long, c_long,
                                c_long, P, c_long, c_int, c_long, P]),
    'wn_reduce_slabs_mt': (c_int, [P, c_int, c_long, c_long, P, c_long, P, c_int,
                                   c_long, c_int, P]),
    'wn_reduce_pair_slabs': (c_int, [P, c_int, c_int, c_int, c_int, c_int, P,
                                     c_int, c_long, c_int, c_int, P]),
    'wn_transpose': (c_int, [P, c_int, c_int, c_long, P, c_long, P]),
    'wn_xent_partials': (c_int, [c_long]),
    'wn_xent': (c_int, [P, c_long, P, P, P, c_int, c_int, c_int, c_int, P]),
    'wn_xent_masked': (c_int, [P, c_long, P, P, P, P, P, c_int, c_int, c_int,
                               c_int, P]),
    'wn_xent_window': (c_int, [P, c_long, P, P, P, P, P, P, c_int, c_int,
                               c_int, c_int, P]),
    'wn_xent_score_window': (c_int, [P, c_long, P, P, P, P, P, P, P, P, c_int,
                                     c_int, c_int, P]),
    'wn_xent_score_scratch_floats': (c_long, [c_long]),
    'wn_xent_score': (c_int, [P, c_long, P, P, P, P, P, P, P, c_int, c_int,
                              c_int, P]),
    'wn_softmax64_row': (c_int, [P, c_int, P, P]),
    'wn_adam': (c_int, [P, P, P, P, c_long, c_float, c_float, c_float,
                        c_float, c_float, c_float, P, P]),
    'wn_momentum': (c_int, [P, P, P, c_long, c_float, c_float, c_float,
                            c_float, P, P]),
    'wn_rmsprop': (c_int, [P, P, P, P, c_long, c_float, c_float, c_float,
                           c_float, c_float, c_float, P, P]),
    'wn_grad_norm_partials_count': (c_int, []),
    'wn_grad_norm_partials': (c_int, [P, c_long, P, P]),
    'wn_adam_clip': (c_int, [P, P, P, P, c_long, c_float, c_float, c_float,
                             c_float, c_float, c_float, P, P, c_int, c_float,
                             P, c_float, P, P]),
    'wn_momentum_clip': (c_int, [P, P, P, c_long, c_float, c_float, c_float,
                                 c_float, P, P, c_int, c_float, P, c_float, P,
                                 P]),
    'wn_rmsprop_clip': (c_int, [P, P, P, P, c_long, c_float, c_float, c_float,
                                c_float, c_float, c_float, P, P, c_int,
                                c_float, P, c_float, P, P]),
    'wn_l2_partials_count': (c_int, []),
    'wn_l2_partials': (c_int, [P, c_long, P, P, P]),
    'wn_gc_bias': (c_int, [P, c_long, c_long, c_long, c_int, P, c_int, P, P,
                           c_int, c_int, c_int, P]),
    'wn_colsum_clip_chunks': (c_int, [c_int]),
    'wn_colsum_clip': (c_int, [P, P, c_int, c_int, P, P, P]),
    'wn_gc_grad': (c_int, [P, c_long, c_long, c_int, P, c_int, P, P, c_int,
                           c_int, P, P, P, c_int, P]),
    'wn_causal_conv': (c_int, [P, P, P, c_int, c_int, c_int, c_int, c_int,
                               c_int, P]),
    'wn_time_to_batch': (c_int, [P, P, c_int, c_int, c_int, c_int, P]),
    'wn_batch_to_time': (c_int, [P, P, c_int, c_int, c_int, c_int, P]),
    'wn_diag_mfma_peak': (c_int, [P, c_int, c_int, P]),
    'wn_axpy': (c_int, [P, P, c_float, P, c_long, P]),
    'wn_fill': (c_int, [P, c_long, c_float, P]),
    'wn_sum_rows': (c_int, [P, c_int, c_int, P, P]),
    'wn_fastgen_state_floats': (c_long, [P, c_int]),
    'wn_fastgen_init': (c_int, [P, c_long, P, c_int, P]),
    'wn_fastgen_run': (c_int, [P, P, c_long, P, P, P, P, P, P, P, P, c_int,
                               c_int, c_int, P, P, P, c_int, c_int, c_float,
                               c_u64, P, c_int, c_int, c_int, P]),
    'wn_fastgen_run_wide': (c_int, [P, P, c_long, P, P, P, P, P, P, P, P,
                                    c_int, c_int, c_int, c_int, P, P, P, c_int,
                                    c_int, c_float, c_u64, P, c_int, c_int,
                                    c_int, P, P]),
    'wn_fastgen_wide_coop_bytes': (c_long, [c_int, c_int, c_int, c_int]),
    'wn_fastgen_step': (c_int, [P, P, c_long, P, P, P, P, P, P, P, P, c_int,
                                c_int, c_int, P, P, P, P, P, c_int, P, P, P,
                                P, P, P, P]),
    'wn_fastgen_persist_workgroups': (c_int, [c_int, c_int, c_int]),
    'wn_fastgen_persist_role': (c_int, [c_int, c_int, c_int]),
    'wn_fastgen_persist_ll_words': (c_long, [c_int, c_int, c_int]),
    'wn_fastgen_persist': (c_int, [P, P, c_long, P, P, P, P, P, P, P, P, c_int,
                                   c_int, c_int, P, P, P, P, P, c_int, P, P, P,
                                   P, P, P, P, P, c_int, P]),
    'wn_fastgen_pre': (c_int, [P, c_long, P, P, c_int, P, P, P, P]),
    'wn_fastgen_finish': (c_int, [c_int, P, P, P, P, P, P]),
    'wn_fastgen_pack': (c_int, [P, c_long, P, c_int, P]),
    'wn_fastgen_batch_rows': (c_int, [c_int]),
    'wn_fastgen_batch_state_floats': (c_long, [P, c_int, c_int]),
    'wn_fastgen_batch_init': (c_int, [P, c_long, P, P, c_int, P]),
    'wn_fastgen_batch_pre': (c_int, [P, c_long, P, c_int, P, c_int, c_int, P,
                                     P, P, P]),
    'wn_fastgen_batch_step': (c_int, [P, P, c_long, P, P, P, P, P, P, P,
                                      c_int, P, c_int, c_int, c_int, c_int, P,
                                      P, P, P, P, P, P, c_int, P, P, P, P, P,
                                      P]),
    'wn_fastgen_batch_stages': (c_int, [c_int, c_int, P, P, c_long, P, P, P,
                                        P, P, P, P, c_int, P, c_int, c_int,
                                        c_int, c_int, P, P, P, P, P, P, P,
                                        c_int, P, P, P, P, P, P]),
    'wn_fastgen_batch_finish': (c_int, [c_int, c_int, P, P, P, P, P, P, P]),
    'wn_fastgen_lc_bias': (c_int, [P, c_long, c_int, P, c_int, P, c_int,
                                   c_int, c_long, c_int, P, c_int, c_int, P]),
    'wn_lc_upsample_floats': (c_int, [P, c_int, c_int]),
    'wn_lc_upsample_fwd': (c_int, [P, c_int, P, P, P, c_int, c_int, c_int, P,
                                   c_int, c_int, c_int, P]),
    'wn_lc_upsample_bwd_slabs': (c_int, [c_long, c_int]),
    'wn_lc_upsample_bwd': (c_int, [P, c_int, P, P, P, c_int, c_int, c_int, P,
                                   c_int, c_int, c_int, P, c_int, c_long, P]),
    'wn_lc_upsample_bwd_ctx': (c_int, [P, c_int, P, P, P, c_int, c_int, c_int,
                                       P, c_int, c_int, c_int, P, c_int,
                                       c_long, P, P, P]),
    'wn_lc_context_fwd': (c_int, [P, c_int, P, c_int, c_int, P, c_int, c_int,
                                  P]),
    'wn_lc_context_wgrad_slabs': (c_int, [c_long, c_int]),
    'wn_lc_context_wgrad': (c_int, [P, c_int, P, c_int, c_int, c_int, c_int, P,
                                    c_int, c_long, P]),
    'wn_melspec': (c_int, [P, c_long, c_int, c_int, P, P, P, P, c_int, c_int,
                           c_int, c_int, c_float, P, P]),
    'wn_feature_stats_partials_count': (c_int, []),
    'wn_feature_stats': (c_int, [P, c_int, c_int, c_int, P, P, P, P]),
    'wn_feature_normalize': (c_int, [P, P, c_int, c_int, c_int, P, P, P,
                                     c_float, c_float, P]),
    'wn_feature_distance_partials': (c_long, [c_int, c_int]),
    'wn_feature_distance': (c_int, [P, P, c_int, c_int, c_int, P, P, P, P, P,
                                    P]),
    'wn_emphasis_chunk': (c_int, []),
    'wn_preemphasis': (c_int, [P, P, c_long, c_long, c_int, c_int, P, c_float,
                               P]),
    'wn_deemphasis': (c_int, [P, P, c_long, c_long, c_int, c_int, P, P, P,
                              c_float, P]),
    'wn_corpus_window_frames': (c_long, [c_int, c_int, c_int]),
    'wn_corpus_gather': (c_int, [P, c_long, P, P, c_int, P, P, c_int, P,
                                 c_long, c_int, c_long, c_int, c_int, c_u64,
                                 P, c_int, c_int, P]),
    'wn_corpus_gather_frames': (c_int, [P, c_long, P, P, P, P, c_int, P, P,
                                        c_int, P, c_long, c_int, c_long,
                                        c_int, c_int, c_u64, c_int, c_int,
                                        c_int, P, c_int, P, c_int, c_int, P]),
    'wn_corpus_gather_hist': (c_int, [P, c_long, P, P, c_int, P, P, c_int, P,
                                      c_long, c_int, c_long, c_int, c_int,
                                      c_u64, c_int, P, P, P, c_int, c_int,
                                      P]),
    'wn_corpus_gather_frames_hist': (c_int, [P, c_long, P, P, P, P, c_int, P,
                                             P, c_int, P, c_long, c_int,
                                             c_long, c_int, c_int, c_u64,
                                             c_int, c_int, c_int, c_int, P,
                                             c_int, P, c_int, c_int, P]),
}
for _name in ('wn_fastgen_run', 'wn_fastgen_pre', 'wn_fastgen_step',
              'wn_fastgen_persist', 'wn_fastgen_batch_pre',
              'wn_fastgen_batch_step'):
    _res, _args = SIGNATURES[_name]
    SIGNATURES[_name + '_lc'] = (_res, _args[:-1] + [P, c_int, c_int, P])
for _name in ('wn_fastgen_run', 'wn_fastgen_run_wide', 'wn_fastgen_run_lc'):
    _res, _args = SIGNATURES[_name]
    SIGNATURES[_name + '_trunc'] = (_res, _args[:-1] + [c_int, c_float, P])



_lib = None


class WaveNetHipError(RuntimeError):
    pass


def load():
    global _lib
    if _lib is not None:
        return _lib
    if not os.path.exists(LIB_PATH):
        raise WaveNetHipError(
            'libwavenet_hip.so not found at %s: build it with '
            '`python __graft_entry__.py build` (hipcc --offload-arch=gfx950). '
            'There is no CPU fallback.' % LIB_PATH)
    lib = ctypes.CDLL(LIB_PATH)
    for name, (res, args) in SIGNATURES.items():
        fn = getattr(lib, name)
        fn.restype = res
        fn.argtypes = args
    _lib = lib
    return lib


def check(code, what=''):
    if code != 0:
        lib = load()
        msg = lib.wn_error_string(int(code)).decode()
        raise WaveNetHipError('%s failed: %s (code %d)' % (what, msg, code))


_rec = None


class record(object):

    def __enter__(self):
        global _rec
        self._outer = _rec
        self.plan = []
        _rec = self.plan
        return self

    def __exit__(self, *exc):
        global _rec
        _rec = self._outer
        return False


def call(name, *args):
    lib = load()
    fn = getattr(lib, name)
    if _rec is not None:
        _rec.append((fn, args, name, None))
    code = fn(*args)
    if code != 0:
        check(code, name)


def call_py(fn):
    def wrapped():
        fn()
        return 0
    if _rec is not None:
        _rec.append((wrapped, (), 'py', None))
    wrapped()


def call_timed(name, args, flops, events):
    lib = load()
    fn = getattr(lib, name)
    if _rec is not None:
        _rec.append((fn, args, name, flops))
    _timed(fn, args, name, flops, events)


def _timed(fn, args, name, flops, events):
    if events is None:
        code = fn(*args)
    else:
        import torch
# ... 42 lines not shown
```

tensorflow-wavenet_amd/wavenet/fastgen.py:

```python
import functools
import warnings

import numpy as np
import torch

from . import _lib
from . import local_condition as lcond
from . import sampling
from . import train_pass

CH = 32
_EXPIRED = dict(
    coop='wn_fastgen_run_wide: a hand-over wait inside the cooperative '
         'generation launch expired (2 s: its workgroups were not all '
         'resident); state restored, continuing with the single workgroup '
         '(net.fastgen_wide_coop = False selects it up front)',
    persist='wn_fastgen_persist: a hand-over wait inside the persistent '
            'generation launch expired (2 s: its workgroups were not all '
            'resident); state restored, continuing with the step kernels '
            '(net.fastgen_persistent = False selects them up front)')


def _new_state(net, dil, nfl, rows, nbias, **extra):
    f32 = dict(dtype=torch.float32, device=net.device)
# ... 108 lines not shown
        _lib.call('wn_sum_rows', _lib.ptr(net._seg(P, 'skip_b')), net.L,
                  net.S, _lib.ptr(g['bsum']), _lib.stream())
        bsum = g['bsum']
    w = (_lib.ptr(net._seg(P, 'causal')), _lib.ptr(net._layer_block(P, 0)),
         net.layer_stride, _lib.ptr(net._seg(P, 'skip_w')), _lib.ptr(bsum),
         _lib.ptr(net._seg(P, 'post1_w')),
         _lib.ptr(net._seg(P, 'post1_b')) if ub else None,
         _lib.ptr(net._seg(P, 'post2_w')),
         _lib.ptr(net._seg(P, 'post2_b')) if ub else None)
    return w, _lib.ptr(bias), bstride


def _stage(net, g, io, n_given, n_steps, temperature, proba, proba_every,
           seed=None, trunc=_NO_TRUNC):
    B, ld = io.shape[0], int(n_steps) + 1
    pe = max(1, int(proba_every))
    rows = (int(n_steps) + pe - 1) // pe if proba is not None else 0
    iob = _buf(net, g, 'io_buf', B * ld, torch.int32)
    iob[:B * ld].view(B, ld).copy_(io[:, :ld])
    pb = None
    if proba is not None:
        pb = _buf(net, g, 'proba_buf', B * rows * net.Q, torch.float32)
    ctl = np.zeros(8, np.uint32)
    ctl[0], ctl[1], ctl[2] = g['steps'], int(n_given), pe
    ctl[3] = np.float32(temperature).view(np.uint32)
    ctl[4], ctl[5] = (ld, rows) if seed is None else \
        (seed & 0xffffffff, seed >> 32)
    ctl[6], ctl[7] = trunc[0], np.float32(trunc[1]).view(np.uint32)
    g['ctl'].copy_(torch.from_numpy(ctl.view(np.int32)))
    return iob, pb


def _replay_steps(net, g, key, one, n_steps):
    def graph_of(nsteps):
        gr = g['graphs'].get((key, nsteps))
        if gr is None:
            gr = torch.cuda.CUDAGraph()
            with torch.cuda.graph(gr):
                for _ in range(nsteps):
                    one()
            if len(g['graphs']) > 8:
                g['graphs'].clear()
            g['graphs'][key, nsteps] = gr
        return gr
    done = 0
    if not g['warm']:
        one()
        done, g['warm'] = 1, True
    for per in (int(net.fastgen_graph_steps),
                max(1, int(net.fastgen_graph_steps) // 10)):
        if per > 1 and n_steps - done >= per:
            gr = graph_of(per)
            while n_steps - done >= per:
                gr.replay()
                done += per
    for _ in range(n_steps - done):
        one()


def _expired(net, kind, scratch, restore):
    if int(scratch[12]) == 0:
        return False
    warnings.warn(_EXPIRED[kind])
    for t, saved in restore:
        t.copy_(saved)
    net._gen_launch_failed[kind] = True
    return True


def _prime(net, g, n0, groups, Bp):
    CB = net.CB
    src, dst, roff = [], [], 0
    for l, d in enumerate(net.dilations):
        t = np.arange(max(0, n0 - d), n0, dtype=np.int64)
        for cb in range(CB):
            src.append((l * CB + cb) * n0 + t)
            dst.append((roff + t % d) * CB + cb)
        roff += d
    src = torch.from_numpy(np.concatenate(src)).to(net.device)
    dst = np.concatenate(dst)
    ws = net._workspace(1, n0, False)
    for codes, gc, streams, lc in groups:
        ws.q.copy_(codes)
        lcond.fill(net, lc, ws)
        train_pass.run_pass(net, 'fwd', ws, net._gc_ids(gc, 1),
                            train_pass.step_path(net, ws, False))
        vals = ws.X.reshape(-1, CH).index_select(0, src) + ws.loss_parts[0]
        rows = dst[None, :] * Bp + np.asarray(streams, np.int64)[:, None]
        g['state'].view(-1, CH).index_copy_(
            0, torch.from_numpy(rows.reshape(-1)).to(net.device),
            vals.repeat(len(streams), 1))


def _seeded(net, io, n_given, n, pe, prime, run, lc=None):
    n_steps = n_given - 1 + n
    primed = prime and pe == 0 and \
        n_given - 1 >= net.fastgen_prime_forward_min and n > 0 and \
        (lc is None or lcond.forward_ok(net, n_given - 1))
    if lc is not None:
        run = functools.partial(run, lc=lc[..., n_given - 1:, :] if primed
                                else lc)
    proba = None
    if pe > 0:
        proba = torch.empty(io.shape[:-1] + ((n_steps + pe - 1) // pe, net.Q),
                            dtype=torch.float32, device=net.device)
    if primed:
        prime()
        tail = io[..., n_given - 1:].clone()
        run(tail, 1, n, None, 1)
        io[..., n_given - 1:] = tail
    elif n_steps > 0:
        run(io, n_given, n_steps, proba, max(1, pe))
    return proba


def generator(net, global_condition):
    if net.CHn > net.FASTGEN_MAX_CHANNELS:
        raise NotImplementedError(
            'fast (incremental) generation supports at most %d residual / '
            'dilation channels on the HIP path; predict_proba (generate.py '
            'without --fast_generation) has no such limit'
            % net.FASTGEN_MAX_CHANNELS)
    if net._gen is None:
        dil = np.asarray(net.dilations, dtype=np.int32)
        nfl = _lib.load().wn_fastgen_state_floats(dil.ctypes.data,
                                                  net.L) * net.CB
        f32 = dict(dtype=torch.float32, device=net.device)
        net._gen = _new_state(
            net, dil, nfl, 1, 1, cw_img=torch.zeros(net.L * 3072, **f32),
            proba=torch.empty(net.Q, **f32),
            io=torch.zeros(2, dtype=torch.int32, device=net.device))
        reset(net)
    return net._gen


def reset(net):
    g = net._gen
    _lib.call('wn_fastgen_init', _lib.ptr(g['state']), g['state'].numel(),
              _lib.ptr(g['cursors']), net.L, _lib.stream())
    g['steps'] = 0


def run(net, temperature, seed, global_condition, samples_io, n_given,
        n_steps, proba_out, proba_every, push=True, multi_cu=False, lc=None,
        trunc=_NO_TRUNC):
    _check_temperature(temperature)
    if int(n_given) < 1:
        raise ValueError('n_given must be >= 1, got %r' % (n_given,))
    g = generator(net, global_condition)
    w, bias, _ = _weights(net, g, global_condition, 1)
    head = w + (bias, _lib.ptr(g['dil']))
    queues = (_lib.ptr(g['state']), _lib.ptr(g['cursors']))
    sd = int(seed) & (2**64 - 1)
    ub = 1 if net.use_biases else 0
    run_args = queues + (_lib.ptr(samples_io), int(n_given), int(n_steps),
                         float(temperature), sd, _lib.ptr(proba_out),
                         int(proba_every), ub, 1 if push else 0)
    if lc is not None:
        _run_lc(net, g, head, bias, queues, samples_io, int(n_given),
                int(n_steps), float(temperature), sd, proba_out,
                max(1, int(proba_every)), ub, push, multi_cu, lc, trunc)
    elif net.CB > 1 or net.S > 512 or net.Q > 512 or net.L > 64:
        _run_wide(net, g, samples_io,
                  head + (net.L, net.CHn, net.S, net.Q) + run_args, trunc)
    elif not multi_cu or not push:
        name, targs = _trunc_entry('wn_fastgen_run', trunc)
# ... 463 lines not shown
```

tensorflow-wavenet_amd/wavenet/model.py:

```python
import math

import numpy as np
import torch

from . import _lib
from . import fastgen
from . import features
from . import local_condition as lcond
from . import sampling
from . import train_pass
from . import workspace
from .ops import mu_law_encode, mu_law_decode, mu_law_tables
from .workspace import CH



def layer_w(K, C=CH):
    return (2 * K + 1) * C * C


def _align(n, a=32):
    return (n + a - 1) // a * a


# ... 459 lines not shown

    def reset_device_errors(self):
        for ws in self._ws.values():
            for name in ('stack_ctl', 'stack_ctl_b'):
                ctl = getattr(ws, name, None)
                if ctl is not None:
                    ctl[3] = 0
            ws.loss_parts[:2] = 0.0

    def _check_supported(self):
        if self._unsupported:
            raise NotImplementedError(self._unsupported)
        if self.device.type != 'cuda':
            raise _lib.WaveNetHipError(
                'WaveNetModel compute needs an MI355X (device=%s); there is '
                'no CPU fallback' % self.device)

    def _workspace(self, B, T, training):
        return workspace.get(self, B, T, training)

    def _step_path(self, ws, backward, l2=False):
        return train_pass.step_path(self, ws, backward, l2)

    def reserve(self, batch_size, max_samples, training=False):
        self._check_supported()
        return self._workspace(int(batch_size), int(max_samples), training)

    def _gc_ids(self, global_condition, B):
        if self.card is None or global_condition is None:
            if self.G is not None and self.card is not None:
                raise ValueError('model was built with global conditioning; '
                                 'a global_condition id batch is required')
            return None
        ids = global_condition
        if not isinstance(ids, torch.Tensor):
            ids = torch.as_tensor(np.asarray(ids))
        ids = ids.reshape(-1).to(device=self.device, dtype=torch.int32)
        if ids.numel() != B:
            raise ValueError('global_condition has %d ids, batch_size is %d'
                             % (ids.numel(), B))
        return ids.contiguous()

    def upsample_local_condition(self, frames, num_samples, offset=0):
        return lcond.upsample(self, frames, num_samples, offset)

    def local_condition_from_audio(self, spec, audio, lengths=None):
        return features.local_condition_from_audio(self, spec, audio, lengths)

    def _layer_block(self, flat, l):
        o, _ = self.segments['layers']
        return flat[o + l * self.layer_stride: o + (l + 1) * self.layer_stride]

    def encode(self, input_batch, B=None):
        B = self.batch_size if B is None else B
        a = input_batch
        if not isinstance(a, torch.Tensor):
            a = torch.as_tensor(np.asarray(a), dtype=torch.float32)
        a = a.to(device=self.device, dtype=torch.float32).reshape(B, -1)
        return mu_law_encode(a, self.Q)

    def loss(self,
             input_batch,
             global_condition_batch=None,
             l2_regularization_strength=None,
             name='wavenet',
             backward=True,
             *,
             local_condition_batch=None,
             local_condition_offset=0,
             lengths=None,
             loss_denominator=None,
             history=None):
        self._check_supported()
        B = self.batch_size
        a = input_batch
        if not isinstance(a, torch.Tensor):
            a = torch.as_tensor(np.asarray(a), dtype=torch.float32)
        a = a.to(device=self.device, dtype=torch.float32).reshape(B, -1)
        mask = check_lengths(lengths, loss_denominator, B, a.shape[1], 'loss')
        mask, hist = check_history(history, mask, loss_denominator, B,
                                   a.shape[1], 'loss')
        lc = lcond.check(self, local_condition_batch, local_condition_offset,
                         B, a.shape[1], 'loss')
        return self._loss(mu_law_encode(a, self.Q), global_condition_batch,
                          l2_regularization_strength, backward, a, lc, mask,
                          hist)

    def loss_from_codes(self, q, global_condition_batch=None,
                        l2_regularization_strength=None, backward=True,
                        audio=None, *, local_condition_batch=None,
                        local_condition_offset=0, lengths=None,
                        loss_denominator=None, history=None):
        self._check_supported()
        q = q.reshape(self.batch_size, -1)
        mask = check_lengths(lengths, loss_denominator, self.batch_size,
                             q.shape[1], 'loss')
        mask, hist = check_history(history, mask, loss_denominator,
                                   self.batch_size, q.shape[1], 'loss')
        lc = lcond.check(self, local_condition_batch, local_condition_offset,
                         self.batch_size, q.shape[1], 'loss')
        return self._loss(q, global_condition_batch,
                          l2_regularization_strength, backward, audio, lc,
                          mask, hist)

    def _loss(self, q, global_condition_batch, l2_regularization_strength,
              backward, audio, lc, mask=None, hist=None):
        B, T = q.shape
        N = B * T
        ws = self._workspace(B, T, backward)
        if backward and self._tail_work is not None:
            import warnings
            from . import parallel
            warnings.warn('the tail all-reduce of the previous backward pass '
                          'was never joined (no optimizer.minimize followed): '
                          'joined and dropped now')
            parallel.abandon_tail_allreduce(self)
        ws.q.copy_(q.reshape(-1))
        if self.scalar_input:
            if audio is None:
                raise ValueError('scalar_input needs the float audio')
            ws.audio.copy_(audio.reshape(-1))
        ids = self._gc_ids(global_condition_batch, B)
        st = _lib.stream()
        lcond.fill(self, lc, ws)
        path = train_pass.step_path(
            self, ws, backward, l2=l2_regularization_strength is not None)
        train_pass.run_pass(self, 'fwd', ws, ids, path)
        quirk = 1 if self.tf_xent_zero_label_quirk else 0
        if mask is None:
            den = float(N)
            _lib.call('wn_xent', _lib.ptr(ws.logits), self.Q, _lib.ptr(ws.q),
                      _lib.ptr(ws.logits) if backward else None,
                      _lib.ptr(ws.loss_parts[2:]), B, T, self.Q, quirk, st)
        else:
            lengths, den = mask
            inv = np.float32(1.0) / np.float32(den)
            ws.xent_mask.copy_(torch.from_numpy(np.concatenate(
                [lengths, np.array([inv], np.float32).view(np.int32)])))
            if hist is None:
                _lib.call('wn_xent_masked', _lib.ptr(ws.logits), self.Q,
                          _lib.ptr(ws.q), _lib.ptr(ws.xent_mask),
                          _lib.ptr(ws.xent_mask[B:]),
                          _lib.ptr(ws.logits) if backward else None,
                          _lib.ptr(ws.loss_parts[2:]), B, T, self.Q, quirk,
                          st)
            else:
                ws.xent_hist.copy_(torch.from_numpy(hist))
                _lib.call('wn_xent_window', _lib.ptr(ws.logits), self.Q,
                          _lib.ptr(ws.q), _lib.ptr(ws.xent_hist),
                          _lib.ptr(ws.xent_mask), _lib.ptr(ws.xent_mask[B:]),
                          _lib.ptr(ws.logits) if backward else None,
                          _lib.ptr(ws.loss_parts[2:]), B, T, self.Q, quirk,
                          st)
        _lib.call('wn_reduce_slabs', _lib.ptr(ws.loss_parts), ws.nparts + 2, 1, 1,
                  0, 0, 1, _lib.ptr(ws.loss), 0, 1, 0, st)
        loss = ws.loss[0] / den
        if backward:
            try:
                train_pass.run_pass(self, 'bwd', ws, ids, path)
            except BaseException:
                from . import parallel
                parallel.abandon_tail_allreduce(self)
                raise
            loss = loss + ws.loss_parts[1]
        if l2_regularization_strength is not None:
            lam = float(l2_regularization_strength)
            mask = None if self.tf_bias_name_quirk else self._l2_mask()
            _lib.call('wn_l2_partials', _lib.ptr(self.params),
                      self.params.numel(), _lib.ptr(mask),
                      _lib.ptr(ws.l2_parts) if backward else
                      _lib.ptr(self._l2_tmp()), st)
            parts = ws.l2_parts if backward else self._l2_tmp()
            loss = loss + lam * parts.sum()
            if backward:
                _lib.call('wn_axpy', _lib.ptr(self.grads),
                          _lib.ptr(self.params), lam, _lib.ptr(mask),
                          self.params.numel(), st)
        loss._wn_model = self
        loss._wn_has_grads = bool(backward)
        return loss

    def score(self, input_batch, global_condition_batch=None, *,
              local_condition_batch=None, local_condition_offset=0,
              lengths=None, per_sample=False, history=None):
        self._check_supported()
        a = input_batch
        if not isinstance(a, torch.Tensor):
            a = torch.as_tensor(np.asarray(a), dtype=torch.float32)
        B = a.shape[0] if a.dim() == 2 and a.shape[0] >= 1 \
            else self.batch_size
        a = a.to(device=self.device, dtype=torch.float32).reshape(B, -1)
        mask = check_lengths(lengths, None, B, a.shape[1], 'score')
        mask, hist = check_history(history, mask, None, B, a.shape[1],
                                   'score')
        lc = lcond.check(self, local_condition_batch, local_condition_offset,
                         B, a.shape[1], 'score')
        from . import scoring
        return scoring.score(self, mu_law_encode(a, self.Q),
                             global_condition_batch, a, lc, mask, per_sample,
                             hist)

    def score_from_codes(self, q, global_condition_batch=None, audio=None, *,
                         local_condition_batch=None, local_condition_offset=0,
                         lengths=None, per_sample=False, history=None):
        self._check_supported()
        if not isinstance(q, torch.Tensor):
            q = torch.as_tensor(np.asarray(q))
        B = q.shape[0] if q.dim() == 2 and q.shape[0] >= 1 \
            else self.batch_size
        q = q.reshape(B, -1)
        mask = check_lengths(lengths, None, B, q.shape[1], 'score')
        mask, hist = check_history(history, mask, None, B, q.shape[1],
                                   'score')
        lc = lcond.check(self, local_condition_batch, local_condition_offset,
                         B, q.shape[1], 'score')
        from . import scoring
        return scoring.score(self, q, global_condition_batch, audio, lc, mask,
                             per_sample, hist)

    def _l2_tmp(self):
        if not hasattr(self, '_l2_parts'):
            self._l2_parts = torch.empty(_lib.load().wn_l2_partials_count(),
                                         dtype=torch.float32,
                                         device=self.device)
        return self._l2_parts

    def _l2_mask(self):
        if not hasattr(self, '_l2m'):
            m = torch.ones_like(self.params)
            tree = self._views(m)
            for n, v in self.named_variables(tree):
                if 'bias' in n.split('/')[-1]:
                    v.zero_()
            self._l2m = m
        return self._l2m

    def predict_proba(self, waveform, global_condition=None, name='wavenet',
                      *, local_condition=None):
        self._check_supported()
        B = self.batch_size
        w = waveform
        if not isinstance(w, torch.Tensor):
            w = torch.as_tensor(np.asarray(w))
        w = w.to(device=self.device, dtype=torch.int32).reshape(B, -1)
        T = w.shape[1]
        lc = lcond.rows(self, local_condition, B, T, 'predict_proba')
        ws = self._workspace(B, T, False)
        ws.q.copy_(w.reshape(-1))
        if self.scalar_input:
            ws.audio.copy_(mu_law_decode(w, self.Q).reshape(-1))
        ids = self._gc_ids(global_condition, B)
        lcond.fill(self, lc, ws)
        train_pass.run_pass(self, 'fwd', ws, ids,
                            train_pass.step_path(self, ws, False))
        out = torch.empty(self.Q, dtype=torch.float32, device=self.device)
        _lib.call('wn_softmax64_row', _lib.ptr(ws.logits[B * T - 1]), self.Q,
                  _lib.ptr(out), _lib.stream())
        return out + ws.loss_parts[0]

    FASTGEN_MAX_CHANNELS = 1024
    FASTGEN_BATCH_MAX = 256

    def predict_proba_incremental(self, waveform, global_condition=None,
                                  name='wavenet', push=True, *,
                                  local_condition=None):
        lc = local_condition
        if self.Lc and lc is not None and np.ndim(lc) == 1:
            lc = lc.reshape(1, -1) if isinstance(lc, torch.Tensor) \
                else np.asarray(lc).reshape(1, -1)
        lc = lcond.fastgen_rows(self, lc, 'predict_proba_incremental', 1)
        return fastgen.predict_proba_incremental(self, waveform,
                                                 global_condition, push, lc)

    def reset_generator(self):
        lcond.refuse_fastgen(self, 'reset_generator')
        fastgen.generator(self, None)
        fastgen.reset(self)

    def generate(self, num_samples, seed_samples=None, temperature=1.0,
                 global_condition=None, seed=0, return_proba_every=0, *,
                 local_condition=None, top_k=None, top_p=None):
        sampling.check(top_k, top_p)
        lc = None
        if self.Lc or local_condition is not None:
            lc = lcond.fastgen_rows(self, local_condition, 'generate',
                                    _n_codes(seed_samples) + int(num_samples)
                                    - 1)
        return fastgen.generate(self, num_samples, seed_samples, temperature,
                                global_condition, seed, return_proba_every,
                                lc, top_k, top_p)

    def prime_generator(self, codes, global_condition=None, *,
                        local_condition=None):
        lc = lcond.fastgen_rows(self, local_condition, 'prime_generator',
                                _n_codes(codes))
        if lc is not None and lc.shape[0] > 0 and \
                not lcond.forward_ok(self, lc.shape[0]):
            raise NotImplementedError(
                'prime_generator: the forward pass that primes an LC model '
                'is the persistent stack launch (wn_stack_fwd_lc): '
                + self.LC_SUPPORTED + ', fewer than 2^24 codes')
        fastgen.prime(self, codes, global_condition, lc)

    def continue_generation(self, num_samples, last_sample, temperature=1.0,
                            global_condition=None, seed=0, *,
                            local_condition=None, top_k=None, top_p=None):
        sampling.check(top_k, top_p)
        lc = lcond.fastgen_rows(self, local_condition, 'continue_generation',
                                int(num_samples))
        return fastgen.continue_generation(self, num_samples, last_sample,
                                           temperature, global_condition, seed,
                                           lc, top_k, top_p)

    def generate_batch(self, num_samples, seeds, seed_samples=None,
                       temperature=1.0, global_condition=None,
                       return_proba_every=0, *, local_condition=None,
                       top_k=None, top_p=None):
        sampling.check(top_k, top_p)
        if self.Lc and local_condition is None:
            lcond.refuse_fastgen(self, 'generate_batch')
        return fastgen.generate_batch(self, num_samples, seeds, seed_samples,
                                      temperature, global_condition,
                                      return_proba_every, local_condition,
                                      top_k, top_p)

    def continue_generation_batch(self, num_samples, last_samples, seeds,
                                  temperature=1.0, global_condition=None,
                                  return_proba_every=0, *,
                                  local_condition=None, top_k=None,
                                  top_p=None):
        sampling.check(top_k, top_p)
# ... 7 lines not shown
```

tensorflow-wavenet_amd/wavenet/scoring.py:

```python
import collections

import torch

from . import _lib
from . import local_condition as lcond
from . import train_pass

Score = collections.namedtuple('Score', 'nll count correct per_sample')


def score(net, q, global_condition_batch, audio, lc, mask, per_sample,
          hist=None):
    B, T = q.shape
    ws = net._workspace(B, T, False)
    ws.q.copy_(q.reshape(-1))
    if net.scalar_input:
        if audio is None:
            raise ValueError('scalar_input needs the float audio')
        ws.audio.copy_(audio.reshape(-1))
    ids = net._gc_ids(global_condition_batch, B)
    lcond.fill(net, lc, ws)
    train_pass.run_pass(net, 'fwd', ws, ids,
                        train_pass.step_path(net, ws, False))
    dev = net.device
    nll = torch.empty(B, dtype=torch.float64, device=dev)
    count = torch.empty(B, dtype=torch.int32, device=dev)
    correct = torch.empty(B, dtype=torch.int32, device=dev)
    rows = torch.empty((B, T), dtype=torch.float32, device=dev) \
        if per_sample else None
    if getattr(ws, 'score_scratch', None) is None:
        ws.score_scratch = torch.empty(
            int(_lib.load().wn_xent_score_scratch_floats(B * T)),
            dtype=torch.float32, device=dev)
    lengths = None
    if mask is not None:
        lengths = ws.xent_mask[:B]
        lengths.copy_(torch.from_numpy(mask[0]))
    if hist is None:
        _lib.call('wn_xent_score', _lib.ptr(ws.logits), net.Q,
                  _lib.ptr(ws.q), _lib.ptr(lengths), _lib.ptr(rows),
                  _lib.ptr(nll), _lib.ptr(count), _lib.ptr(correct),
                  _lib.ptr(ws.score_scratch), B, T, net.Q, _lib.stream())
    else:
        ws.xent_hist.copy_(torch.from_numpy(hist))
        _lib.call('wn_xent_score_window', _lib.ptr(ws.logits), net.Q,
                  _lib.ptr(ws.q), _lib.ptr(ws.xent_hist), _lib.ptr(lengths),
                  _lib.ptr(rows), _lib.ptr(nll), _lib.ptr(count),
                  _lib.ptr(correct), _lib.ptr(ws.score_scratch), B, T, net.Q,
                  _lib.stream())
    return Score(nll + ws.loss_parts[0], count, correct, rows)
```

tensorflow-wavenet_amd/wavenet/train_pass.py:

```python
import collections

import torch

from . import _lib
from . import local_condition as lcond
from .workspace import CH

TN_SIDE_SPLIT_FRAC = 0.6

StepPath = collections.namedtuple('StepPath', [
    'fwd', 'save_ts', 'bwd', 'pack_both', 'overlap_tn', 'early_allreduce',
    'causal_wgrad', 'gemm_mode', 'variant'])


def step_path(net, ws, backward, l2=False):
    layers, lc = net._layer_path(), '_lc' if net.Lc else ''
    fwd = layers
    if net.stack_fwd and net._stack_ok():
        skip = (net.stack_fwd_skip and net.gemm_mode == 'fp32' and
                not net.residual_postproc and ws.fwd_skip_ok)
        fwd = 'stack_skip' if skip else 'stack' + lc
    if not backward:
        return StepPath(fwd, 0, None, False, False, False, None,
                        net.gemm_mode, ws.stack_variant)
    bwd = layers
    if layers == 'layer':
        bwd = 'stack' + lc if net._stack_bwd_ok() and ws.stack_bwd \
            else 'layer2'
    if net.Lc and bwd != 'stack_lc':
        raise NotImplementedError(net.LC_SUPPORTED)
    from . import parallel
    early = bool(net.dp_overlap_allreduce and not l2 and
                 parallel.is_distributed())
    causal = (None if layers == 'blocked' else 'scalar' if net.scalar_input
              else 'segsum' if net.KW == 2 and net.Q <= 256 else 'onehot')
    return StepPath(fwd, 2 if layers == 'layer' else 1, bwd,
                    fwd.startswith('stack') and bwd.startswith('stack'),
                    net._overlap_tn_on(ws), early, causal,
                    net.gemm_mode, ws.stack_variant)


def early_allreduce(net):
    from . import parallel
    _lib.call_py(lambda: parallel.begin_tail_allreduce(net))


def side_stream(net):
    if getattr(net, '_side', None) is None:
        net._side = torch.cuda.Stream(device=net.device, priority=0)
    return net._side


def bias_fg(net, ws_bias, ids, B):
    if not net.use_biases and ids is None:
        return None, 0
    nb = B if ids is not None else 1
    W2 = 2 * net.CHn
    out = ws_bias.view(-1)[:net.L * nb * W2].view(net.L, nb, W2)
    emb = net._seg(net.params, 'emb') if ids is not None else None
    _lib.call('wn_gc_bias', _lib.ptr(net._layer_block(net.params, 0)),
              net.layer_stride, net.OFF_BF, net.OFF_GC, net.G or 0,
              _lib.ptr(emb), net.card or 0, _lib.ptr(ids), _lib.ptr(out),
              net.L, nb, net.CHn, _lib.stream())
    return out, (W2 if ids is not None else 0)


def nn_seq(net, calls):
    st = _lib.stream()
    for c in calls:
        nn(net, *(c + (st,)))


def nn(net, *args):
    name = 'wn_gemm_nn'
    if net.gemm_mode != 'fp32':
        nprod = {'bf16x3': 3, 'bf16x6': 6, 'bf16x9': 9}[net.gemm_mode]
        M, N, K = args[-5], args[-4], args[-3]
        if K % 16 == 0:
            key = (args[4], K, N)
            buf = net._wsplit.get(key)
            if buf is None:
                nb = _lib.load().wn_gemm_split_w_bytes(K, N)
                buf = torch.empty(nb // 4, dtype=torch.int32,
                                  device=net.device)
                net._wsplit[key] = buf
            name = 'wn_gemm_nn_split'
            args = args[:-1] + (_lib.ptr(buf), nprod, args[-1])
    k = -7 if name == 'wn_gemm_nn_split' else -5
    _lib.call_timed(name, args, 2.0 * args[k] * args[k + 1] * args[k + 2],
                    net._gemm_events)


def stage_ids(net, ws, ids):
    if ids is None:
        return None
    if ids.data_ptr() != ws.gc_ids.data_ptr():
        ws.gc_ids.copy_(ids)
    return ws.gc_ids


def run_pass(net, tag, ws, ids, path):
    eager = forward_eager if tag == 'fwd' else backward_eager
    ids = stage_ids(net, ws, ids)
    if not net.use_launch_plans or (tag == 'bwd' and path.bwd == 'blocked'):
        return eager(net, ws, ids, path)
    key = (tag, path, ids is not None, _lib.stream(),
           net.params.data_ptr(), net.grads.data_ptr())
    plan = ws.plans.get(key, 0)
    if plan == 0:
        ws.plans[key] = None
        eager(net, ws, ids, path)
    elif plan is None:
        with _lib.record() as rec:
            eager(net, ws, ids, path)
        ws.plans[key] = rec.plan
    else:
        _lib.replay(plan, net._gemm_events)


def forward_eager(net, ws, ids, path):
    st = _lib.stream()
    B, T, N, L, S, Q = ws.B, ws.T, ws.N, net.L, net.S, net.Q
    P = net.params
    wc = net._seg(P, 'causal')
    for cb in range(net.CB):
        if net.scalar_input:
            _lib.call('wn_scalar_causal_fwd', _lib.ptr(ws.audio),
                      _lib.ptr(wc[cb * CH:]), net.CHn, _lib.ptr(ws.X[cb]),
                      B, T, net.initial_filter_width, st)
        else:
            _lib.call('wn_causal_gather', _lib.ptr(ws.q),
                      _lib.ptr(wc[cb * CH:]), _lib.ptr(ws.X[cb]), B, T, Q,
                      net.KW, net.CHn, st)
    bias, bstride = bias_fg(net, ws.bias_fg, ids, B)
    save_ts = path.save_ts
    if path.fwd == 'blocked':
        from . import blocked
        blocked.forward_layers(net, ws, bias, bstride, bool(save_ts), st)
    elif path.fwd.startswith('stack'):
        fwd_stack(net, ws, path, bias, bstride, st)
    else:
        for l, d in enumerate(net.dilations):
            last = l == L - 1
            fargs = (_lib.ptr(ws.X[l]),
                     None if last else _lib.ptr(ws.X[l + 1]),
                     _lib.ptr(ws.Z[l]),
                     _lib.ptr(ws.TH[l]) if save_ts == 1 else None,
                     _lib.ptr(ws.SG[l]) if save_ts else None,
                     _lib.ptr(net._layer_block(P, l)),
                     None if bias is None else _lib.ptr(bias[l]), bstride,
                     B, T, int(d))
            if path.fwd == 'layer_k':
                _lib.call('wn_layer_fwd_k', *fargs, net.KW,
                          0 if last else 1, 1 if save_ts else 0, st)
            else:
                _lib.call('wn_layer_fwd', *fargs, 0 if last else 1,
                          int(save_ts), st)
    fuse_skip = path.fwd == 'stack_skip'
    bsum = None
    if net.use_biases and not fuse_skip:
        _lib.call('wn_sum_rows', _lib.ptr(net._seg(P, 'skip_b')), L, S,
                  _lib.ptr(ws.bsum), st)
        bsum = ws.bsum
    LP, C = L * net.CB, net.CHn
    b1 = net._seg(P, 'post1_b') if net.use_biases else None
    b2 = net._seg(P, 'post2_b') if net.use_biases else None
    rp = net.residual_postproc
    skip_gemm = [] if fuse_skip else [
        (_lib.ptr(ws.Z), 0, LP, N * CH,
         _lib.ptr(net._seg(P, 'skip_w')), S, _lib.ptr(bsum), None, 0,
         None, 0, _lib.ptr(ws.h1), S, 0, 0,
         _lib.ptr(ws.total) if net.residual_postproc else None,
         N, S, L * C, 1)]
    nn_seq(net, skip_gemm + [
        (_lib.ptr(ws.h1), S, 0, 0,
         _lib.ptr(net._seg(P, 'post1_w')), S, _lib.ptr(b1), None, 0,
         _lib.ptr(ws.total) if rp else None, S, _lib.ptr(ws.h2), S, 0,
         0, _lib.ptr(ws.c1) if (rp and ws.training) else None,
         N, S, S, 1),
        (_lib.ptr(ws.h2), S, 0, 0,
         _lib.ptr(net._seg(P, 'post2_w')), Q, _lib.ptr(b2), None, 0,
         None, 0, _lib.ptr(ws.logits), Q, 0, 0, None, N, Q, S, 0)])


def fwd_stack(net, ws, path, bias, bstride, st):
    B, T, N, L, S = ws.B, ws.T, ws.N, net.L, net.S
    P = net.params
    _lib.call('wn_stack_pack', _lib.ptr(net._layer_block(P, 0)),
              net.layer_stride, _lib.ptr(ws.wimg_f),
              _lib.ptr(ws.wimg_b) if path.pack_both else None, L, st)
    save = path.save_ts != 0
    stack_args = (_lib.ptr(ws.X), _lib.ptr(ws.Z),
                  _lib.ptr(ws.SG) if save else None,
                  _lib.ptr(ws.wimg_f),
                  None if bias is None else _lib.ptr(bias),
                  0 if bias is None else bias.shape[1] * bias.shape[2],
                  bstride, _lib.ptr(net._dil_dev),
                  _lib.ptr(ws.stack_flags), _lib.ptr(ws.stack_ctl),
                  _lib.ptr(ws.loss_parts),
                  L, B, T, 1 if save else 0, ws.stack_variant)
    if path.fwd == 'stack_skip':
        if getattr(ws, 'skimg', None) is None:
            ws.skimg = torch.empty(
                int(_lib.load().wn_stack_skip_img_floats(L)),
                dtype=torch.float32, device=net.device)
        bsum_f = None
        if net.use_biases:
            _lib.call('wn_sum_rows', _lib.ptr(net._seg(P, 'skip_b')), L,
                      S, _lib.ptr(ws.bsum), st)
            bsum_f = ws.bsum
        _lib.call('wn_stack_skip_pack', _lib.ptr(net._seg(P, 'skip_w')),
                  L, _lib.ptr(ws.skimg), st)
        _lib.call_timed('wn_stack_fwd_skip', stack_args + (
            _lib.ptr(ws.skimg), _lib.ptr(bsum_f), _lib.ptr(ws.h1), st),
            0.0, net._gemm_events)
    elif path.fwd == 'stack_lc':
        W64 = L * 64
        _lib.call_timed('wn_gemm_nn', (
            _lib.ptr(ws.lc), net.Lcp, 0, 0,
            _lib.ptr(net._seg(P, 'lc_w')), W64, None, None, 0, None,
            0, _lib.ptr(ws.lc_add), W64, 0, 0, None, N, W64, net.Lcp,
            0, st), 2.0 * N * W64 * net.Lcp, net._gemm_events)
        _lib.call_timed('wn_stack_fwd_lc', stack_args + (
            _lib.ptr(ws.lc_add), W64, st), 0.0, net._gemm_events)
    else:
        _lib.call_timed('wn_stack_fwd', stack_args + (st,), 0.0,
                        net._gemm_events)


def backward_eager(net, ws, ids, path):
    st = _lib.stream()
    bwd_post(net, ws, path, st)
    if path.bwd == 'blocked':
        from . import blocked
        if path.overlap_tn:
            main_s = torch.cuda.current_stream()
            _lib.call_py(lambda: main_s.wait_event(ws.ev_join))
        blocked.backward_layers(net, ws, ids, st)
        return
    run = {'layer2': bwd_layer2,
           'layer_k': bwd_layer_k}.get(path.bwd, bwd_stack)
    backward_tail(net, ws, ids, path, run(net, ws, path, st))


def bwd_post(net, ws, path, st):
    N, L, S, Q = ws.N, net.L, net.S, net.Q
    P, Gr = net.params, net.grads
    rp = net.residual_postproc
    dlog = ws.logits
    LP, C = L * net.CB, net.CHn
    _lib.call('wn_transpose', _lib.ptr(net._seg(P, 'post2_w')), S, Q, Q,
              _lib.ptr(ws.w2t), S, st)
    _lib.call('wn_transpose', _lib.ptr(net._seg(P, 'post1_w')), S, S, S,
              _lib.ptr(ws.w1t), S, st)
    _lib.call('wn_transpose', _lib.ptr(net._seg(P, 'skip_w')), L * C, S,
              S, _lib.ptr(ws.wst), L * C, st)
    nn_dc1 = (_lib.ptr(dlog), Q, 0, 0, _lib.ptr(ws.w2t), S,
              None, _lib.ptr(ws.c1 if rp else ws.h2), S, None, 0,
              _lib.ptr(ws.dc1), S, 0, 0, _lib.ptr(ws.dh2) if rp else None,
              N, S, Q, 0)
    nn_dtotal = (_lib.ptr(ws.dc1), S, 0, 0, _lib.ptr(ws.w1t), S,
                 None, _lib.ptr(ws.h1), S, _lib.ptr(ws.dh2) if rp else None,
                 S, _lib.ptr(ws.dtotal), S, 0, 0, None, N, S, S, 0)
    nn_dz = (_lib.ptr(ws.dtotal), S, 0, 0, _lib.ptr(ws.wst),
             L * C, None, None, 0, None, 0, _lib.ptr(ws.dZ), 0, LP,
             N * CH, None, N, L * C, S, 0)
    tns = [('post2', _lib.ptr(ws.h2), S, 0, 0, _lib.ptr(dlog), Q, S, Q,
            _lib.ptr(net._seg(Gr, 'post2_w')),
            _lib.ptr(net._seg(Gr, 'post2_b'))),
           ('post1', _lib.ptr(ws.h1), S, 0, 0, _lib.ptr(ws.dc1), S, S, S,
            _lib.ptr(net._seg(Gr, 'post1_w')),
            _lib.ptr(net._seg(Gr, 'post1_b'))),
           ('skip', _lib.ptr(ws.Z), 0, LP, N * CH, _lib.ptr(ws.dtotal), S,
            L * C, S, _lib.ptr(net._seg(Gr, 'skip_w')),
            _lib.ptr(net._seg(Gr, 'skip_b')), L, S)]
    if not path.overlap_tn:
        nn_seq(net, [nn_dc1, nn_dtotal, nn_dz])
        for key, *a in tns:
            tn(net, ws, path, st, ws.region[key], *a)
        if path.early_allreduce:
            early_allreduce(net)
        return
    nn_seq(net, [nn_dc1, nn_dtotal])
    main_s = torch.cuda.current_stream()
    side_s = side_stream(net)
    _lib.call_py(lambda: (ws.ev_fork.record(main_s),
                          side_s.wait_event(ws.ev_fork)))
    for key, *a in tns:
        tn(net, ws, path, side_s.cuda_stream, ws.region[key + '_side'], *a)
    _lib.call_py(lambda: ws.ev_join.record(side_s))
    nn(net, *(nn_dz + (st,)))


def reduce_slabs(reg, dst, st, count=None, offset=0, n=None, replicate=1,
                 rep_stride=0):
    _lib.call('wn_reduce_slabs', _lib.ptr(reg.buf),
              reg.count if count is None else count, reg.stride, 1, 0, offset,
              reg.n if n is None else n, dst, 0, replicate, rep_stride, st)


def tn(net, ws, path, st, reg, A, lda, a_planes, a_pstride, Gm, ldg, mw, nw,
       dst, dst_bias, replicate=1, rep_stride=0):
    lib = _lib.load()
    N = ws.N
    ub = 1 if net.use_biases else 0
    sp, sl = reg.count, reg.stride
    if path.overlap_tn and 256 < ws.B * ((ws.T + 31) // 32) <= 512:
        sp = max(1, int(sp * TN_SIDE_SPLIT_FRAC))
    mt = bool(ub and dst_bias is not None and (mw * nw) % 4 == 0 and
              nw % 4 == 0 and sl % 4 == 0 and rep_stride % 4 == 0)
    tr = int(lib.wn_gemm_tn_tail_rows(mw, nw)) \
        if mt and path.gemm_mode == 'fp32' else 1
    if path.gemm_mode != 'fp32' and N % 16 == 0:
        sp = min(sp, lib.wn_gemm_tn_splits(N, mw, nw, 2))
        _lib.call('wn_gemm_tn_split', A, lda, a_planes, a_pstride, Gm,
                  ldg, _lib.ptr(reg.buf), sp, N, mw, nw, ub,
                  int(path.gemm_mode[-1]), st)
    else:
        _lib.call_timed('wn_gemm_tn',
                        (A, lda, a_planes, a_pstride, None, 0, ws.T,
                         Gm, ldg, _lib.ptr(reg.buf), sp, N, mw, nw,
                         2 if tr > 1 else ub,
                         st), 2.0 * N * mw * nw, net._gemm_events)
    if mt:
        _lib.call('wn_reduce_slabs_mt', _lib.ptr(reg.buf), sp, sl,
                  mw * nw, dst, nw, dst_bias, replicate, rep_stride,
                  tr, st)
        return
    reduce_slabs(reg, dst, st, sp)
    if ub and dst_bias is not None:
        reduce_slabs(reg, dst_bias, st, sp, offset=mw * nw, n=nw,
                     replicate=replicate, rep_stride=rep_stride)


def bwd_stack(net, ws, path, st):
    B, T, L = ws.B, ws.T, net.L
    tsum = None if ws.dsum is None else \
        ws.tilesum16 if ws.stack_rows == 16 else ws.tilesum
    if not path.pack_both:
# ... 18 lines not shown
    return ws.DX[0]


def bwd_layer2(net, ws, path, st):
    B, T, L, P = ws.B, ws.T, net.L, net.params
    tsum = None if ws.dsum is None else ws.tilesum
    _lib.call('wn_layer_bwd2_pack', _lib.ptr(net._layer_block(P, 0)),
              net.layer_stride, _lib.ptr(ws.wimg), L, st)
    dxin, xp = None, 0
    for l in range(L - 1, -1, -1):
        dxo = ws.dx[xp]
        _lib.call('wn_layer_bwd2', _lib.ptr(ws.X[l]), _lib.ptr(ws.Z[l]),
                  _lib.ptr(ws.SG[l]), _lib.ptr(ws.dZ[l]),
                  _lib.ptr(dxin), _lib.ptr(dxo),
                  _lib.ptr(net._layer_block(P, l)),
                  _lib.ptr(ws.wimg[l]), _lib.ptr(ws.lslabs[l]),
                  None if tsum is None else _lib.ptr(tsum[l]),
                  B, T, int(net.dilations[l]), st)
        dxin, xp = dxo, 1 - xp
    return dxin


def bwd_layer_k(net, ws, path, st):
    B, T, L, P = ws.B, ws.T, net.L, net.params

    def da(p):
        return ws.da[p][0], ws.da[p][1]

    def layer_bwd(*a):
        _lib.call('wn_layer_bwd_k', *a[:14], net.KW, *a[14:16], 1, 0, a[16])

    def layer_wgrad(*a):
        _lib.call('wn_layer_wgrad_k', *a[:10], net.KW, 0, net.KW, 1, 0, a[10])
    cur = 0
    f, g = da(cur)
    layer_bwd(None, None, None, None, None,
              _lib.ptr(ws.dZ[L - 1]), _lib.ptr(ws.TH[L - 1]),
              _lib.ptr(ws.SG[L - 1]),
              _lib.ptr(net._layer_block(P, L - 1)), _lib.ptr(f),
              _lib.ptr(g), B, T, 1, 0, 1, st)
    dxin, xp = None, 0
    for l in range(L - 1, -1, -1):
        d = int(net.dilations[l])
        f, g = da(cur)
        dxo = ws.dx[xp]
        layer_wgrad(_lib.ptr(ws.X[l]), _lib.ptr(f), _lib.ptr(g),
                    None if dxin is None else _lib.ptr(ws.Z[l]),
                    None if dxin is None else _lib.ptr(dxin),
                    _lib.ptr(ws.lslabs[l]), ws.region['layers_k'].count, B, T,
                    d, st)
        if ws.dsum is not None:
            _lib.call('wn_colsum_clip', _lib.ptr(f), _lib.ptr(g), B, T,
                      _lib.ptr(ws.dsum_part), _lib.ptr(ws.dsum[l]), st)
        if l > 0:
            fn, gn = da(1 - cur)
            layer_bwd(_lib.ptr(f), _lib.ptr(g),
                      None if dxin is None else _lib.ptr(dxin),
                      _lib.ptr(dxo), _lib.ptr(net._layer_block(P, l)),
                      _lib.ptr(ws.dZ[l - 1]), _lib.ptr(ws.TH[l - 1]),
                      _lib.ptr(ws.SG[l - 1]),
                      _lib.ptr(net._layer_block(P, l - 1)), _lib.ptr(fn),
                      _lib.ptr(gn), B, T, d, 1, 1, st)
            cur = 1 - cur
        else:
            layer_bwd(_lib.ptr(f), _lib.ptr(g),
                      None if dxin is None else _lib.ptr(dxin),
                      _lib.ptr(dxo), _lib.ptr(net._layer_block(P, l)),
                      None, None, None, None, None, None, B, T, d, 1, 0,
                      st)
        dxin, xp = dxo, 1 - xp
    return dxin


def backward_tail(net, ws, ids, path, dxin):
    if path.overlap_tn:
        main_s = torch.cuda.current_stream()
        _lib.call_py(lambda: main_s.wait_event(ws.ev_join))
        if path.early_allreduce:
            early_allreduce(net)
    st = _lib.stream()
    B, T, N, L, Q = ws.B, ws.T, ws.N, net.L, net.Q
    P, Gr = net.params, net.grads
    stack = path.bwd.startswith('stack')
    if path.bwd != 'layer_k' and ws.dsum is not None:
        tile_rows = ws.stack_rows if stack else 32
        tpc = (T + tile_rows - 1) // tile_rows
        _lib.call('wn_reduce_slabs', _lib.ptr(ws.tilesum), tpc, 64, L * B,
                  tpc * 64, 0, 64, _lib.ptr(ws.dsum), 64, 1, 0, st)
    reg = ws.region['layers_stack' if stack else
                    'layers_2' if path.bwd == 'layer2' else 'layers_k']
    lo, _ = net.segments['layers']
    _lib.call('wn_reduce_slabs', _lib.ptr(reg.buf), reg.count, reg.stride, L,
              ws.lslabs.shape[1] * reg.stride, 0, reg.n, _lib.ptr(Gr[lo:]),
              net.layer_stride, 1, 0, st)
    gc_ = net._seg(Gr, 'causal')
    if path.causal_wgrad == 'scalar':
        reg = ws.region['causal_scalar']
        _lib.call('wn_scalar_causal_wgrad', _lib.ptr(ws.audio),
                  _lib.ptr(dxin), _lib.ptr(reg.buf), reg.count, B, T,
                  net.initial_filter_width, st)
        reduce_slabs(reg, _lib.ptr(gc_), st)
    elif path.causal_wgrad == 'segsum':
        reg = ws.region['causal_segsum']
        _lib.call('wn_causal_wgrad', _lib.ptr(ws.q), _lib.ptr(dxin),
                  _lib.ptr(reg.buf), reg.count, B, T, Q, st)
        reduce_slabs(reg, _lib.ptr(gc_), st)
    else:
        K, reg = net.KW, ws.region['causal_onehot']
        for tap in range(K):
            shift = (K - 1 - tap) + (K - 1) // 2
            _lib.call('wn_gemm_tn', None, 0, 0, 0, _lib.ptr(ws.q), shift,
                      T, _lib.ptr(dxin), CH, _lib.ptr(reg.buf), reg.count, N,
                      Q, CH, 0, st)
            reduce_slabs(reg, _lib.ptr(gc_[tap * Q * CH:]), st)
    if net.Lc:
        lcond.backward(net, ws, st)
    if ws.dsum is not None:
        _lib.call('wn_gc_grad', _lib.ptr(net._layer_block(P, 0)),
                  net.layer_stride, net.OFF_GC, net.G,
                  _lib.ptr(net._seg(P, 'emb')), net.card, _lib.ptr(ids),
                  _lib.ptr(ws.dsum), L, B,
                  _lib.ptr(net._layer_block(Gr, 0)),
                  _lib.ptr(net._seg(Gr, 'emb')), _lib.ptr(ws.gc_part),
                  net.CHn, st)
```

tensorflow-wavenet_amd/wavenet/workspace.py:

```python
import collections

import numpy as np
import torch

from . import _lib
from . import local_condition as lcond

CH = 32

SlabRegion = collections.namedtuple('SlabRegion', 'buf count stride n')


class _Workspace(object):

    def __init__(self, net, B, T, training, parent=None):
        dev = net.device
        L, S, Q = net.L, net.S, net.Q
        CB, CHn = net.CB, net.CHn
        LP = L * CB
        N = B * T
        self.B, self.T, self.N, self.training = B, T, N, training
        self.stack_variant = net._stack_variant_for_launch()
        self.capacity = N if parent is None else parent.capacity
        lib = _lib.load()
        self.fwd_skip_ok = bool(lib.wn_stack_fwd_skip_ok(B, T, S,
                                                         self.stack_variant))

        def alloc(name, shape, dtype=torch.float32, fill=None):
            n = int(np.prod(shape))
            if parent is not None and getattr(parent, name, None) is not None:
                t = getattr(parent, name).reshape(-1)[:n].view(shape)
            else:
                fresh.add(name)
                if fill is None:
                    t = torch.empty(shape, dtype=dtype, device=dev)
                else:
                    t = torch.full(shape, fill, dtype=dtype, device=dev)
            setattr(self, name, t)
            return t

        fresh = set()

        self.plans = {}
        alloc('q', (N,), torch.int32)
        self.gc_ids = alloc('gc_ids', (B,), torch.int32) \
            if net.card is not None else None
        self.audio = alloc('audio', (N,)) if net.scalar_input else None
        alloc('X', (LP, N, CH))
        alloc('Z', (LP, N, CH))
        alloc('h1', (N, S))
        alloc('h2', (N, S))
        alloc('logits', (N, Q))
        alloc('bias_fg', (L, B, 2 * CHn))
        alloc('stack_flags', (lib.wn_stack_flag_count(B, T, L),), torch.int32,
              fill=0)
        alloc('wimg_f', (L, lib.wn_stack_wimg_floats()))
        alloc('stack_ctl', (4,), torch.int32, fill=0)
        if 'stack_ctl' in fresh:
            self.stack_ctl[2] = 1
        alloc('bsum', (S,))
        self.total = alloc('total', (N, S)) if net.residual_postproc else None
        self.nparts = lib.wn_xent_partials(N)
        alloc('loss_parts', (2 + self.nparts,), fill=0.0)
        alloc('loss', (1,), fill=0.0)
        alloc('xent_mask', (B + 1,), torch.int32, fill=0)
        alloc('xent_hist', (B,), torch.int32, fill=0)
        alloc('proba', (Q,))
        lcond.alloc_workspace(net, self, alloc, None)
        if net.blocked:
            alloc('pre', (2 * CB, N, CH))
        if not training:
            return
        self.legacy = net._layer_path() != 'layer'
        self.TH = alloc('TH', (LP, N, CH)) if self.legacy else None
        alloc('SG', (LP, N, CH))
        alloc('dZ', (LP, N, CH))
        alloc('dc1', (N, S))
        alloc('dtotal', (N, S))
        self.dh2 = alloc('dh2', (N, S)) if net.residual_postproc else None
        self.c1 = alloc('c1', (N, S)) if net.residual_postproc else None
        self.da = alloc('da', (2, 2 * CB, N, CH)) if self.legacy else None
        alloc('dx', (2, CB, N, CH))
        self.stack_bwd = bool(net.stack_bwd and net._stack_ok(N))
        if self.stack_bwd:
            self.keep_dx = bool(net.stack_bwd_keep_dx)
            if parent is not None and getattr(parent, 'DX', None) is not None:
                self.keep_dx = parent.keep_dx
            alloc('DX', (L if self.keep_dx else 1, N, CH))
            alloc('DQ', (L, N, CH))
            alloc('wimg_b', (L, lib.wn_stack_wimg_floats()))
            alloc('stack_flags_b', (lib.wn_stack_flag_count(B, T, L),),
                  torch.int32, fill=0)
            alloc('stack_ctl_b', (4,), torch.int32, fill=0)
            if 'stack_ctl_b' in fresh:
                self.stack_ctl_b[2] = 1
        if net.blocked:
            alloc('dzb', (CB, N, CH))
            alloc('wdT', (CHn, CHn))
            alloc('blk_tmp', (max((2 * net.KW + 1) * 1024 + 96, Q * CH,
                                  net.initial_filter_width * CH),))
            alloc('cs_tmp', (B, 64))
        alloc('w2t', (Q, S))
        alloc('w1t', (S, S))
        alloc('wst', (S, L * CHn))
        shared = []

        def region(key, count, stride, n, own=None, side=False):
            if own:
                self.region[key] = SlabRegion(alloc(own, (count, stride)),
                                              count, stride, n)
            else:
                shared.append((key, count, stride, n, side))

        self.region = {}
        ntiles = B * ((T + 31) // 32)
        nslab = max(1, min(512, ntiles // 4))
        alloc('wimg', (L, lib.wn_layer_bwd2_wimg_floats()))
        if net.blocked:
            pair = (2 * min(net.KW, 8) + 1) * 1024 + 96
            nslab = max(1, min(nslab, (8 << 30) // (CB * CB * pair * 4)))
            alloc('pslabs', (CB * CB, nslab, pair))
            self.region['pairs'] = SlabRegion(self.pslabs, nslab, pair, pair)
            alloc('lslabs', (1, 1, 4))
        else:
            counts = dict(
                layers_k=nslab, layers_2=lib.wn_layer_bwd2_slabs(B, T),
                layers_stack=lib.wn_stack_bwd_slabs(B, T, self.stack_variant)
                if self.stack_bwd else 0)
            fit = _view_stack_slabs(lib, B, T, self.stack_variant) \
                if parent is None and net._stack_ok() else 0
# ... 81 lines not shown
```

Before: 13.55 million.

## Fuse per-step weight packing, transposes, mu-law encode and slab reductions into fewer launches

```diff
diff --git a/include/wavenet_hip.h b/include/wavenet_hip.h
--- a/include/wavenet_hip.h
+++ b/include/wavenet_hip.h
@@ -161,6 +161,19 @@
                     int batch, long in_batch_stride, long offset, long n,
                     float* dst, long out_batch_stride, int replicate,
                     long rep_stride, void* stream);
+#define WN_REDUCE_MAX_JOBS 4
+typedef struct wn_reduce_job {
+  const float* slabs;
+  int num_slabs;
+  long slab_stride;
+  int batch;
+  long in_batch_stride, offset, n;
+  float* dst;
+  long out_batch_stride;
+  int replicate;
+  long rep_stride;
+} wn_reduce_job;
+int wn_reduce_slabs_multi(const wn_reduce_job* jobs, int njobs, void* stream);
 int wn_reduce_slabs_mt(const float* slabs, int num_slabs, long slab_stride,
                        long n_main, float* dst_main, long n_tail, float* dst_tail,
                        int replicate, long rep_stride, int tail_rows, void* stream);
@@ -253,6 +266,13 @@
             void* stream);
 int wn_fill(float* p, long n, float value, void* stream);
 int wn_sum_rows(const float* in, int rows, int n, float* out, void* stream);
+
+int wn_step_prologue(const float* layer0, long layer_stride, float* wimg_fwd,
+                     float* wimg_bwd, int L, const float* post2_w, float* w2t,
+                     const float* post1_w, float* w1t, const float* skip_w,
+                     float* wst, int S, int Q, const float* skip_b, float* bsum,
+                     const float* audio, const float* thr_dev, int32_t* q,
+                     const float* Wc, float* x0, int B, int T, void* stream);
 
 long wn_fastgen_state_floats(const int32_t* dilations_host, int L);
 int wn_fastgen_init(float* state, long state_floats, int32_t* cursors, int L,
diff --git a/tensorflow-wavenet_amd/csrc/wn_gemm.hip b/tensorflow-wavenet_amd/csrc/wn_gemm.hip
--- a/tensorflow-wavenet_amd/csrc/wn_gemm.hip
+++ b/tensorflow-wavenet_amd/csrc/wn_gemm.hip
@@ -1,4 +1,5 @@
 #include "wn_common.h"
+#include "wn_small.inc"
 #include <cstdlib>
 #include <cstddef>
 #include <cstring>
@@ -1252,15 +1253,16 @@
   }
 }
 
-__global__ void reduce_slabs_kernel(const float* __restrict__ slabs,
-                                    int num_slabs, long slab_stride,
-                                    long in_batch_stride, long offset, long n,
-                                    float* __restrict__ dst,
-                                    long out_batch_stride, int replicate,
-                                    long rep_stride) {
-  const long e = (long)blockIdx.x * blockDim.x + threadIdx.x;
+
+__device__ __forceinline__ void reduce_slabs_body(const float* __restrict__ slabs,
+                                                  int num_slabs, long slab_stride,
+                                                  long in_batch_stride, long offset, long n,
+                                                  float* __restrict__ dst,
+                                                  long out_batch_stride, int replicate,
+                                                  long rep_stride, unsigned bx, int b,
+                                                  unsigned bdim, unsigned tid) {
+  const long e = (long)bx * bdim + tid;
   if (e >= n) return;
-  const int b = blockIdx.y;
   const float* p = slabs + (long)b * in_batch_stride + offset + e;
   float s0 = 0.f, s1 = 0.f, s2 = 0.f, s3 = 0.f;
   int s = 0;
@@ -1276,6 +1278,60 @@
     dst[(long)b * out_batch_stride + (long)r * rep_stride + e] = v;
 }
 
+__global__ void reduce_slabs_kernel(const float* __restrict__ slabs,
+                                    int num_slabs, long slab_stride,
+                                    long in_batch_stride, long offset, long n,
+                                    float* __restrict__ dst,
+                                    long out_batch_stride, int replicate,
+                                    long rep_stride) {
+  reduce_slabs_body(slabs, num_slabs, slab_stride, in_batch_stride, offset, n, dst,
+                    out_batch_stride, replicate, rep_stride, blockIdx.x, blockIdx.y,
+                    blockDim.x, threadIdx.x);
+}
+
+template <int PARTS>
+__device__ __forceinline__ void reduce_slabs4_body(f32x4 (*part)[64],
+                                                   const float* __restrict__ slabs,
+                                                   int num_slabs, long slab_stride,
+                                                   long in_batch_stride, long offset, long n4,
+                                                   float* __restrict__ dst,
+                                                   long out_batch_stride, int replicate,
+                                                   long rep_stride, unsigned bx, int b, int tid) {
+  const int col = tid & 63, pt = tid >> 6;
+  const long e = (long)bx * 64 + col;
+  const int per = (num_slabs + PARTS - 1) / PARTS;
+  const int s0 = pt * per, s1 = min(num_slabs, s0 + per);
+  f32x4 acc[8];
+#pragma unroll
+  for (int k = 0; k < 8; ++k) acc[k] = f32x4{0.f, 0.f, 0.f, 0.f};
+  if (e < n4) {
+    const f32x4* p = reinterpret_cast<const f32x4*>(slabs + (long)b * in_batch_stride + offset) + e;
+    const long st = slab_stride / 4;
+    int s = s0;
+    for (; s + 7 < s1; s += 8) {
+      f32x4 v[8];
+#pragma unroll
+      for (int k = 0; k < 8; ++k) v[k] = p[(long)(s + k) * st];
+#pragma unroll
+      for (int k = 0; k < 8; ++k) acc[k] += v[k];
+    }
+#pragma unroll
+    for (int k = 0; k < 7; ++k)
+      if (s + k < s1) acc[k] += p[(long)(s + k) * st];
+  }
+  f32x4 v = ((acc[0] + acc[1]) + (acc[2] + acc[3])) + ((acc[4] + acc[5]) + (acc[6] + acc[7]));
+  if (PARTS > 1) {
+    part[pt][col] = v;
+    __syncthreads();
+    if (pt != 0) return;
+    if (PARTS == 4) v = (part[0][col] + part[1][col]) + (part[2][col] + part[3][col]);
+    else v = part[0][col] + part[1][col];
+  }
+  if (e >= n4) return;
+  for (int r = 0; r < replicate; ++r)
+    *reinterpret_cast<f32x4*>(dst + (long)b * out_batch_stride + (long)r * rep_stride + 4 * e) = v;
+}
+
 template <int PARTS>
 __global__ void reduce_slabs4_kernel(const float* __restrict__ slabs,
                                      int num_slabs, long slab_stride,
@@ -1284,40 +1340,9 @@
                                      long out_batch_stride, int replicate,
                                      long rep_stride) {
   __shared__ f32x4 part[PARTS > 1 ? PARTS : 1][64];
-  const int col = threadIdx.x & 63, pt = threadIdx.x >> 6;
-  const long e = (long)blockIdx.x * 64 + col;
-  const int b = blockIdx.y;
-  const int per = (num_slabs + PARTS - 1) / PARTS;
-  const int s0 = pt * per, s1 = min(num_slabs, s0 + per);
-  f32x4 acc[8];
-#pragma unroll
-  for (int k = 0; k < 8; ++k) acc[k] = f32x4{0.f, 0.f, 0.f, 0.f};
-  if (e < n4) {
-    const f32x4* p = reinterpret_cast<const f32x4*>(slabs + (long)b * in_batch_stride + offset) + e;
-    const long st = slab_stride / 4;
-    int s = s0;
-    for (; s + 7 < s1; s += 8) {
-      f32x4 v[8];
-#pragma unroll
-      for (int k = 0; k < 8; ++k) v[k] = p[(long)(s + k) * st];
-#pragma unroll
-      for (int k = 0; k < 8; ++k) acc[k] += v[k];
-    }
-#pragma unroll
-    for (int k = 0; k < 7; ++k)
-      if (s + k < s1) acc[k] += p[(long)(s + k) * st];
-  }
-  f32x4 v = ((acc[0] + acc[1]) + (acc[2] + acc[3])) + ((acc[4] + acc[5]) + (acc[6] + acc[7]));
-  if (PARTS > 1) {
-    part[pt][col] = v;
-    __syncthreads();
-    if (pt != 0) return;
-    if (PARTS == 4) v = (part[0][col] + part[1][col]) + (part[2][col] + part[3][col]);
-    else v = part[0][col] + part[1][col];
-  }
-  if (e >= n4) return;
-  for (int r = 0; r < replicate; ++r)
-    *reinterpret_cast<f32x4*>(dst + (long)b * out_batch_stride + (long)r * rep_stride + 4 * e) = v;
+  reduce_slabs4_body<PARTS>(part, slabs, num_slabs, slab_stride, in_batch_stride, offset, n4,
+                            dst, out_batch_stride, replicate, rep_stride, blockIdx.x,
+                            blockIdx.y, threadIdx.x);
 }
 
 #ifndef RMT_PARTS
@@ -1438,17 +1463,7 @@
                                      int cols, long in_ld,
                                      float* __restrict__ out, long out_ld) {
   __shared__ float tile[32][33];
-  const int bx = blockIdx.x * 32, by = blockIdx.y * 32;
-  const int tx = threadIdx.x & 31, ty = threadIdx.x >> 5;
-  for (int k = ty; k < 32; k += 8) {
-    const int r = by + k, c = bx + tx;
-    tile[k][tx] = (r < rows && c < cols) ? in[(long)r * in_ld + c] : 0.f;
-  }
-  __syncthreads();
-  for (int k = ty; k < 32; k += 8) {
-    const int c = bx + k, r = by + tx;
-    if (c < cols && r < rows) out[(long)c * out_ld + r] = tile[tx][k];
-  }
+  transpose_pad_body(tile, in, rows, cols, in_ld, out, out_ld, blockIdx.x, blockIdx.y);
 }
 
 template <int MODE>
@@ -1750,20 +1765,97 @@
   return wn_check_launch();
 }
 
+__device__ __forceinline__ void reduce_slabs_wave_body(
+    const float* __restrict__ slabs, int num_slabs, long slab_stride,
+    long in_batch_stride, long offset, float* __restrict__ dst,
+    long out_batch_stride, int replicate, long rep_stride, unsigned bx, int b, int lane) {
+  const long e = bx;
+  const float* p = slabs + (long)b * in_batch_stride + offset + e;
+  float v = 0.f;
+  for (int s = lane; s < num_slabs; s += 64) v += p[(long)s * slab_stride];
+#pragma unroll
+  for (int o = 32; o >= 1; o >>= 1) v += __shfl_xor(v, o);
+  if (lane == 0)
+    for (int r = 0; r < replicate; ++r)
+      dst[(long)b * out_batch_stride + (long)r * rep_stride + e] = v;
+}
+
 __global__ __launch_bounds__(64) void reduce_slabs_wave_kernel(
     const float* __restrict__ slabs, int num_slabs, long slab_stride,
     long in_batch_stride, long offset, float* __restrict__ dst,
     long out_batch_stride, int replicate, long rep_stride) {
-  const long e = blockIdx.x;
-  const int b = blockIdx.y;
-  const float* p = slabs + (long)b * in_batch_stride + offset + e;
-  float v = 0.f;
-  for (int s = threadIdx.x; s < num_slabs; s += 64) v += p[(long)s * slab_stride];
-#pragma unroll
-  for (int o = 32; o >= 1; o >>= 1) v += __shfl_xor(v, o);
-  if (threadIdx.x == 0)
-    for (int r = 0; r < replicate; ++r)
-      dst[(long)b * out_batch_stride + (long)r * rep_stride + e] = v;
+  reduce_slabs_wave_body(slabs, num_slabs, slab_stride, in_batch_stride, offset, dst,
+                         out_batch_stride, replicate, rep_stride, blockIdx.x, blockIdx.y,
+                         threadIdx.x);
+}
+
+#define WN_REDUCE_MAX_JOBS 4
+struct wn_reduce_job {
+  const float* slabs;
+  int num_slabs;
+  long slab_stride;
+  int batch;
+  long in_batch_stride, offset, n;
+  float* dst;
+  long out_batch_stride;
+  int replicate;
+  long rep_stride;
+};
+enum { RK_WAVE = 0, RK_VEC4 = 1, RK_VEC1 = 2, RK_SCALAR = 3 };
+struct ReduceJob {
+  const float* slabs;
+  float* dst;
+  long slab_stride, in_batch_stride, offset, n, out_batch_stride, rep_stride;
+  int num_slabs, batch, replicate, kind;
+  unsigned gx;
+};
+struct ReduceMulti {
+  ReduceJob job[WN_REDUCE_MAX_JOBS];
+  unsigned start[WN_REDUCE_MAX_JOBS + 1];
+};
+
+static int reduce_slabs_kind(const float* slabs, int num_slabs, long slab_stride,
+                             int batch, long in_batch_stride, long offset, long n,
+                             const float* dst, long out_batch_stride, long rep_stride) {
+  if (n <= 4 && num_slabs >= 256) return RK_WAVE;
+  if (((n | offset | slab_stride | in_batch_stride | out_batch_stride | rep_stride) & 3) == 0 &&
+      wn_aligned16(slabs) && wn_aligned16(dst)) {
+    const long gx = (n / 4 + 63) / 64;
+    return num_slabs >= 32 && gx * batch <= 4096 ? RK_VEC4 : RK_VEC1;
+  }
+  return RK_SCALAR;
+}
+
+__global__ __launch_bounds__(256) void reduce_slabs_multi_kernel(ReduceMulti m) {
+  __shared__ f32x4 part[4][64];
+  int j = 0;
+#pragma unroll
+  for (int k = 1; k < WN_REDUCE_MAX_JOBS; ++k)
+    if (blockIdx.x >= m.start[k]) j = k;
+  const ReduceJob& g = m.job[j];
+  const unsigned lb = blockIdx.x - m.start[j];
+  const int tid = threadIdx.x;
+  if (g.kind == RK_VEC4) {
+    reduce_slabs4_body<4>(part, g.slabs, g.num_slabs, g.slab_stride, g.in_batch_stride,
+                          g.offset, g.n, g.dst, g.out_batch_stride, g.replicate, g.rep_stride,
+                          lb % g.gx, lb / g.gx, tid);
+  } else if (g.kind == RK_SCALAR) {
+    reduce_slabs_body(g.slabs, g.num_slabs, g.slab_stride, g.in_batch_stride, g.offset, g.n,
+                      g.dst, g.out_batch_stride, g.replicate, g.rep_stride, lb % g.gx,
+                      lb / g.gx, 256, tid);
+  } else {
+    const unsigned ob = 4 * lb + (tid >> 6);
+    const unsigned by = ob / g.gx;
+    if (by >= (unsigned)g.batch) return;
+    if (g.kind == RK_VEC1)
+      reduce_slabs4_body<1>(part, g.slabs, g.num_slabs, g.slab_stride, g.in_batch_stride,
+                            g.offset, g.n, g.dst, g.out_batch_stride, g.replicate,
+                            g.rep_stride, ob % g.gx, by, tid & 63);
+    else
+      reduce_slabs_wave_body(g.slabs, g.num_slabs, g.slab_stride, g.in_batch_stride, g.offset,
+                             g.dst, g.out_batch_stride, g.replicate, g.rep_stride, ob % g.gx,
+                             by, tid & 63);
+  }
 }
 
 int wn_reduce_slabs(const float* slabs, int num_slabs, long slab_stride,
@@ -1799,6 +1891,51 @@
   hipLaunchKernelGGL(reduce_slabs_kernel, grid, block, 0, (hipStream_t)stream,
                      slabs, num_slabs, slab_stride, in_batch_stride, offset, n,
                      dst, out_batch_stride, replicate, rep_stride);
+  return wn_check_launch();
+}
+
+int wn_reduce_slabs_multi(const wn_reduce_job* jobs, int njobs, void* stream) {
+  if (!jobs) return WN_ERR_NULL;
+  if (njobs <= 0) return WN_ERR_BAD_SHAPE;
+  if (njobs > WN_REDUCE_MAX_JOBS) return WN_ERR_UNSUPPORTED;
+  ReduceMulti m;
+  memset(&m, 0, sizeof(m));
+  unsigned long total = 0;
+  for (int j = 0; j < njobs; ++j) {
+    const wn_reduce_job& a = jobs[j];
+    if (!a.slabs || !a.dst) return WN_ERR_NULL;
+    if (a.num_slabs <= 0 || a.n <= 0 || a.batch <= 0 || a.replicate <= 0)
+      return WN_ERR_BAD_SHAPE;
+    if ((reinterpret_cast<uintptr_t>(a.slabs) | reinterpret_cast<uintptr_t>(a.dst)) & 3u)
+      return WN_ERR_MISALIGNED;
+    ReduceJob& g = m.job[j];
+    g.slabs = a.slabs;
+    g.dst = a.dst;
+    g.slab_stride = a.slab_stride;
+    g.in_batch_stride = a.in_batch_stride;
+    g.offset = a.offset;
+    g.out_batch_stride = a.out_batch_stride;
+    g.rep_stride = a.rep_stride;
+    g.num_slabs = a.num_slabs;
+    g.batch = a.batch;
+    g.replicate = a.replicate;
+    g.kind = reduce_slabs_kind(a.slabs, a.num_slabs, a.slab_stride, a.batch, a.in_batch_stride,
+                               a.offset, a.n, a.dst, a.out_batch_stride, a.rep_stride);
+    const bool vec = g.kind == RK_VEC4 || g.kind == RK_VEC1;
+    g.n = vec ? a.n / 4 : a.n;
+    const unsigned long gx = g.kind == RK_WAVE ? (unsigned long)a.n
+                             : vec ? (unsigned long)((g.n + 63) / 64)
+                                   : (unsigned long)((a.n + 255) / 256);
+    unsigned long wgs = gx * (unsigned long)a.batch;
+    if (g.kind == RK_WAVE || g.kind == RK_VEC1) wgs = (wgs + 3) / 4;
+    if (gx > 0x7fffffffUL || total + wgs > 0x7fffffffUL) return WN_ERR_BAD_SHAPE;
+    g.gx = (unsigned)gx;
+    m.start[j] = (unsigned)total;
+    total += wgs;
+  }
+  for (int j = njobs; j <= WN_REDUCE_MAX_JOBS; ++j) m.start[j] = (unsigned)total;
+  hipLaunchKernelGGL(reduce_slabs_multi_kernel, dim3((unsigned)total), dim3(256), 0,
+                     (hipStream_t)stream, m);
   return wn_check_launch();
 }
 
diff --git a/tensorflow-wavenet_amd/csrc/wn_misc.hip b/tensorflow-wavenet_amd/csrc/wn_misc.hip
--- a/tensorflow-wavenet_amd/csrc/wn_misc.hip
+++ b/tensorflow-wavenet_amd/csrc/wn_misc.hip
@@ -1,5 +1,7 @@
 #include "wn_common.h"
+#include "wn_small.inc"
 #include <stdlib.h>
+#include <string.h>
 #include <cmath>
 
 #pragma clang fp contract(off)
@@ -46,6 +48,21 @@
   return (int)v;
 }
 
+__device__ __forceinline__ int mu_law_code_dev(float x, const float* sthr, int Q) {
+  int code;
+  if (x >= -1.f && x <= 1.f) {
+    int lo = 0, hi = Q - 1;
+    while (lo < hi) {
+      const int mid = (lo + hi) >> 1;
+      if (sthr[mid] <= x) lo = mid + 1; else hi = mid;
+    }
+    code = lo;
+  } else {
+    code = mu_chain_dev(x, Q);
+  }
+  return code;
+}
+
 __global__ void mu_law_encode_kernel(const float* __restrict__ audio,
                                      int32_t* __restrict__ codes, long n,
                                      const float* __restrict__ thr, int Q) {
@@ -53,21 +70,8 @@
   for (int i = threadIdx.x; i < Q - 1; i += blockDim.x) sthr[i] = thr[i];
   __syncthreads();
   for (long idx = (long)blockIdx.x * blockDim.x + threadIdx.x; idx < n;
-       idx += (long)gridDim.x * blockDim.x) {
-    const float x = audio[idx];
-    int code;
-    if (x >= -1.f && x <= 1.f) {
-      int lo = 0, hi = Q - 1;
-      while (lo < hi) {
-        const int mid = (lo + hi) >> 1;
-        if (sthr[mid] <= x) lo = mid + 1; else hi = mid;
-      }
-      code = lo;
-    } else {
-      code = mu_chain_dev(x, Q);
-    }
-    codes[idx] = code;
-  }
+       idx += (long)gridDim.x * blockDim.x)
+    codes[idx] = mu_law_code_dev(audio[idx], sthr, Q);
 }
 
 __device__ __forceinline__ float mu_decode_dev(int code, int Q) {
@@ -87,6 +91,28 @@
     const int c = codes[idx];
     audio[idx] = (c >= 0 && c < Q) ? lut[c] : mu_decode_dev(c, Q);
   }
+}
+
+struct CodesInMemory {
+  const int32_t* __restrict__ q;
+  __device__ __forceinline__ int operator()(long r) const { return q[r]; }
+};
+template <typename CodeAt>
+__device__ __forceinline__ void causal_gather_row(CodeAt code_at,
+                                                  const float* __restrict__ Wc,
+                                                  float* __restrict__ x0, long row, int c4,
+                                                  int T, int Q, int K, int ldw) {
+  const int t = (int)(row % T);
+  f32x4 v = {0.f, 0.f, 0.f, 0.f};
+  const int extra = (K - 1) / 2;
+  for (int k = 0; k < K; ++k) {
+    const int s = (K - 1 - k) + extra;
+    if (t < s) continue;
+    const int code = code_at(row - s);
+    if (code >= 0 && code < Q)
+      v += *reinterpret_cast<const f32x4*>(Wc + ((long)k * Q + code) * ldw + c4);
+  }
+  *reinterpret_cast<f32x4*>(x0 + row * 32 + c4) = v;
 }
 
 __global__ void causal_gather_kernel(const int32_t* __restrict__ q,
@@ -97,17 +123,7 @@
   const long row = idx >> 3;
   const int c4 = (idx & 7) * 4;
   if (row >= rows) return;
-  const int t = (int)(row % T);
-  f32x4 v = {0.f, 0.f, 0.f, 0.f};
-  const int extra = (K - 1) / 2;
-  for (int k = 0; k < K; ++k) {
-    const int s = (K - 1 - k) + extra;
-    if (t < s) continue;
-    const int code = q[row - s];
-    if (code >= 0 && code < Q)
-      v += *reinterpret_cast<const f32x4*>(Wc + ((long)k * Q + code) * ldw + c4);
-  }
-  *reinterpret_cast<f32x4*>(x0 + row * 32 + c4) = v;
+  causal_gather_row(CodesInMemory{q}, Wc, x0, row, c4, T, Q, K, ldw);
 }
 
 __global__ void scalar_causal_fwd_kernel(const float* __restrict__ audio,
@@ -317,9 +333,8 @@
     p[i] = v;
 }
 
-__global__ void sum_rows_kernel(const float* __restrict__ in, int rows, int n,
-                                float* __restrict__ out) {
-  const int c = blockIdx.x * blockDim.x + threadIdx.x;
+__device__ __forceinline__ void sum_rows_body(const float* __restrict__ in, int rows, int n,
+                                              float* __restrict__ out, int c) {
   if (c >= n) return;
   float s = 0.f;
   int r = 0;
@@ -332,6 +347,79 @@
   }
   for (; r < rows; ++r) s += in[(long)r * n + c];
   out[c] = s;
+}
+
+__global__ void sum_rows_kernel(const float* __restrict__ in, int rows, int n,
+                                float* __restrict__ out) {
+  sum_rows_body(in, rows, n, out, blockIdx.x * blockDim.x + threadIdx.x);
+}
+
+enum { PJ_PACK_F = 0, PJ_PACK_B, PJ_GATHER, PJ_BSUM, PJ_TRANSPOSE, PJ_COUNT = PJ_TRANSPOSE + 3 };
+struct StepPrologue {
+  const float* layer0;
+  long layer_stride;
+  float* img_f;
+  float* img_b;
+  const float* tin[3];
+  float* tout[3];
+  int trows[3], tcols[3];
+  unsigned tgx[3];
+  const float* skip_b;
+  float* bsum;
+  int L, S;
+  const float* audio;
+  const float* thr;
+  int32_t* q;
+  const float* Wc;
+  float* x0;
+  long rows;
+  int T, Q;
+  unsigned start[PJ_COUNT + 1];
+};
+#define PROLOGUE_GATHER_ROWS 32
+
+__global__ __launch_bounds__(256) void step_prologue_kernel(StepPrologue a) {
+  extern __shared__ float smem[];
+  int j = 0;
+#pragma unroll
+  for (int k = 1; k < PJ_COUNT; ++k)
+    if (blockIdx.x >= a.start[k]) j = k;
+  const unsigned lb = blockIdx.x - a.start[j];
+  const int tid = threadIdx.x;
+  if (j == PJ_PACK_F) {
+    stack_pack_body(a.layer0, a.layer_stride, a.img_f, lb, false);
+  } else if (j == PJ_PACK_B) {
+    stack_pack_body(a.layer0, a.layer_stride, a.img_b, lb, true);
+  } else if (j == PJ_BSUM) {
+    sum_rows_body(a.skip_b, a.L, a.S, a.bsum, lb * 256 + tid);
+  } else if (j >= PJ_TRANSPOSE) {
+    const int t = j - PJ_TRANSPOSE;
+    transpose_pad_body(reinterpret_cast<float(*)[33]>(smem), a.tin[t], a.trows[t], a.tcols[t],
+                       a.tcols[t], a.tout[t], a.trows[t], lb % a.tgx[t], lb / a.tgx[t]);
+  } else {
+    const long row0 = (long)lb * PROLOGUE_GATHER_ROWS;
+    const long row = row0 + (tid >> 3);
+    const int c4 = (tid & 7) * 4;
+    if (a.audio) {
+      float* sthr = smem;
+      int* scode = reinterpret_cast<int*>(smem + (a.Q - 1));
+      for (int i = tid; i < a.Q - 1; i += 256) sthr[i] = a.thr[i];
+      __syncthreads();
+      const long r = row0 - 1 + tid;
+      if (tid <= PROLOGUE_GATHER_ROWS && r >= 0 && r < a.rows) {
+        const int code = mu_law_code_dev(a.audio[r], sthr, a.Q);
+        scode[tid] = code;
+        if (tid >= 1) a.q[r] = code;
+      }
+      __syncthreads();
+      if (row >= a.rows) return;
+      causal_gather_row([scode, row0](long rr) { return scode[(int)(rr - row0) + 1]; }, a.Wc,
+                        a.x0, row, c4, a.T, a.Q, 2, 32);
+    } else {
+      if (row >= a.rows) return;
+      causal_gather_row(CodesInMemory{a.q}, a.Wc, a.x0, row, c4, a.T, a.Q, 2, 32);
+    }
+  }
 }
 
 extern "C" {
@@ -678,4 +766,68 @@
   return wn_check_launch();
 }
 
-}
+int wn_step_prologue(const float* layer0, long layer_stride, float* wimg_fwd,
+                     float* wimg_bwd, int L, const float* post2_w, float* w2t,
+                     const float* post1_w, float* w1t, const float* skip_w,
+                     float* wst, int S, int Q, const float* skip_b, float* bsum,
+                     const float* audio, const float* thr_dev, int32_t* q,
+                     const float* Wc, float* x0, int B, int T, void* stream) {
+  if (!layer0 || !wimg_fwd || !q || !Wc || !x0) return WN_ERR_NULL;
+  if ((w2t && !post2_w) || (w1t && !post1_w) || (wst && !skip_w) || (bsum && !skip_b) ||
+      (audio && !thr_dev))
+    return WN_ERR_NULL;
+  if (L <= 0 || layer_stride < LAYER_BLOCK_FLOATS || B <= 0 || T <= 0 || S <= 0 || Q < 2 ||
+      Q > 8192)
+    return WN_ERR_BAD_SHAPE;
+  if (!wn_aligned16(wimg_fwd) || (wimg_bwd && !wn_aligned16(wimg_bwd)) || !wn_aligned16(Wc) ||
+      !wn_aligned16(x0))
+    return WN_ERR_MISALIGNED;
+  StepPrologue a;
+  memset(&a, 0, sizeof(a));
+  a.layer0 = layer0;
+  a.layer_stride = layer_stride;
+  a.img_f = wimg_fwd;
+  a.img_b = wimg_bwd;
+  const float* tin[3] = {post2_w, post1_w, skip_w};
+  float* tout[3] = {w2t, w1t, wst};
+  const int trows[3] = {S, S, L * 32}, tcols[3] = {Q, S, S};
+  a.skip_b = skip_b;
+  a.bsum = bsum;
+  a.L = L;
+  a.S = S;
+  a.audio = audio;
+  a.thr = thr_dev;
+  a.q = q;
+  a.Wc = Wc;
+  a.x0 = x0;
+  a.rows = (long)B * T;
+  a.T = T;
+  a.Q = Q;
+  unsigned long wgs[PJ_COUNT];
+  wgs[PJ_PACK_F] = L;
+  wgs[PJ_PACK_B] = wimg_bwd ? L : 0;
+  wgs[PJ_GATHER] = (a.rows + PROLOGUE_GATHER_ROWS - 1) / PROLOGUE_GATHER_ROWS;
+  wgs[PJ_BSUM] = bsum ? (S + 255) / 256 : 0;
+  for (int t = 0; t < 3; ++t) {
+    a.tin[t] = tin[t];
+    a.tout[t] = tout[t];
+    a.trows[t] = trows[t];
+    a.tcols[t] = tcols[t];
+    a.tgx[t] = (tcols[t] + 31) / 32;
+    wgs[PJ_TRANSPOSE + t] = tout[t] ? (unsigned long)a.tgx[t] * ((trows[t] + 31) / 32) : 0;
+  }
+  unsigned long total = 0;
+  for (int j = 0; j < PJ_COUNT; ++j) {
+    a.start[j] = (unsigned)total;
+    total += wgs[j];
+  }
+  a.start[PJ_COUNT] = (unsigned)total;
+  if (total > 0x7fffffffUL) return WN_ERR_BAD_SHAPE;
+  const size_t lds = sizeof(float) * (size_t)(Q - 1 + PROLOGUE_GATHER_ROWS + 1 > 32 * 33
+                                                  ? Q - 1 + PROLOGUE_GATHER_ROWS + 1 : 32 * 33);
+  hipLaunchKernelGGL(step_prologue_kernel, dim3((unsigned)total), dim3(256), lds,
+                     (hipStream_t)stream, a);
+  return wn_check_launch();
+}
+
+}
diff --git a/tensorflow-wavenet_amd/csrc/wn_small.inc b/tensorflow-wavenet_amd/csrc/wn_small.inc
--- /dev/null
+++ b/tensorflow-wavenet_amd/csrc/wn_small.inc
@@ -0,0 +1,40 @@
+#pragma once
+
+#define SF_LD 36
+#define SF_MT (32 * SF_LD)
+#define SF_OFF_BD (5 * SF_MT)
+#define STACK_WBUF 5888
+
+__device__ __forceinline__ void stack_pack_body(const float* __restrict__ layer0,
+                                                long layer_stride, float* __restrict__ img,
+                                                unsigned layer, bool bwd) {
+  const float* blk = layer0 + (long)layer * layer_stride;
+  float* out = img + (size_t)layer * STACK_WBUF;
+  for (int i = threadIdx.x; i < STACK_WBUF; i += blockDim.x) out[i] = 0.f;
+  __syncthreads();
+  for (int i = threadIdx.x; i < LAYER_W_FLOATS; i += blockDim.x) {
+    const int m = i >> 10, cin = (i >> 5) & 31, cout = i & 31;
+    out[bwd ? m * 1024 + cin * 32 + ((((cout >> 2) ^ ((cin >> 1) & 7)) << 2) | (cout & 3))
+            : m * SF_MT + cout * SF_LD + cin] = blk[i];
+  }
+  if (!bwd && threadIdx.x < 32)
+    out[SF_OFF_BD + threadIdx.x] = blk[LAYER_OFF_BD + threadIdx.x];
+}
+
+__device__ __forceinline__ void transpose_pad_body(float (*tile)[33],
+                                                   const float* __restrict__ in, int rows,
+                                                   int cols, long in_ld,
+                                                   float* __restrict__ out, long out_ld,
+                                                   int tbx, int tby) {
+  const int bx = tbx * 32, by = tby * 32;
+  const int tx = threadIdx.x & 31, ty = threadIdx.x >> 5;
+  for (int k = ty; k < 32; k += 8) {
+    const int r = by + k, c = bx + tx;
+    tile[k][tx] = (r < rows && c < cols) ? in[(long)r * in_ld + c] : 0.f;
+  }
+  __syncthreads();
+  for (int k = ty; k < 32; k += 8) {
+    const int c = bx + k, r = by + tx;
+    if (c < cols && r < rows) out[(long)c * out_ld + r] = tile[tx][k];
+  }
+}
diff --git a/tensorflow-wavenet_amd/csrc/wn_stack.hip b/tensorflow-wavenet_amd/csrc/wn_stack.hip
--- a/tensorflow-wavenet_amd/csrc/wn_stack.hip
+++ b/tensorflow-wavenet_amd/csrc/wn_stack.hip
@@ -4,10 +4,7 @@
 #define WN_WAIT_LGKM0() asm volatile("s_waitcnt lgkmcnt(0)" ::: "memory")
 
 #define STACK_MAXL 256
-#define SF_LD 36
-#define SF_MT (32 * SF_LD)
-#define SF_OFF_BD (5 * SF_MT)
-#define STACK_WBUF 5888
+#include "wn_small.inc"
 
 struct StackFwd {
   float* X;
@@ -128,17 +125,7 @@
   const bool bwd = blockIdx.y == 1;
   float* img = bwd ? img_b : img_f;
   if (!img) return;
-  const float* blk = layer0 + (long)blockIdx.x * layer_stride;
-  float* out = img + (size_t)blockIdx.x * STACK_WBUF;
-  for (int i = threadIdx.x; i < STACK_WBUF; i += blockDim.x) out[i] = 0.f;
-  __syncthreads();
-  for (int i = threadIdx.x; i < LAYER_W_FLOATS; i += blockDim.x) {
-    const int m = i >> 10, cin = (i >> 5) & 31, cout = i & 31;
-    out[bwd ? m * 1024 + cin * 32 + ((((cout >> 2) ^ ((cin >> 1) & 7)) << 2) | (cout & 3))
-            : m * SF_MT + cout * SF_LD + cin] = blk[i];
-  }
-  if (!bwd && threadIdx.x < 32)
-    out[SF_OFF_BD + threadIdx.x] = blk[LAYER_OFF_BD + threadIdx.x];
+  stack_pack_body(layer0, layer_stride, img, blockIdx.x, bwd);
 }
 
 __device__ __forceinline__ void wait_lds(const int* p, bool& dead, unsigned* ctl,
diff --git a/tensorflow-wavenet_amd/wavenet/_lib.py b/tensorflow-wavenet_amd/wavenet/_lib.py
--- a/tensorflow-wavenet_amd/wavenet/_lib.py
+++ b/tensorflow-wavenet_amd/wavenet/_lib.py
@@ -86,6 +86,7 @@
                            c_long, P, c_int, c_long, c_int, c_int, c_int, P]),
     'wn_reduce_slabs': (c_int, [P, c_int, c_long, c_int, c_long, c_long,
                                 c_long, P, c_long, c_int, c_long, P]),
+    'wn_reduce_slabs_multi': (c_int, [P, c_int, P]),
     'wn_reduce_slabs_mt': (c_int, [P, c_int, c_long, c_long, P, c_long, P, c_int,
                                    c_long, c_int, P]),
     'wn_reduce_pair_slabs': (c_int, [P, c_int, c_int, c_int, c_int, c_int, P,
@@ -136,6 +137,9 @@
     'wn_axpy': (c_int, [P, P, c_float, P, c_long, P]),
     'wn_fill': (c_int, [P, c_long, c_float, P]),
     'wn_sum_rows': (c_int, [P, c_int, c_int, P, P]),
+    'wn_step_prologue': (c_int, [P, c_long, P, P, c_int, P, P, P, P, P, P,
+                                 c_int, c_int, P, P, P, P, P, P, P, c_int,
+                                 c_int, P]),
     'wn_fastgen_state_floats': (c_long, [P, c_int]),
     'wn_fastgen_init': (c_int, [P, c_long, P, c_int, P]),
     'wn_fastgen_run': (c_int, [P, P, c_long, P, P, P, P, P, P, P, P, c_int,
@@ -230,6 +234,17 @@
     SIGNATURES[_name + '_trunc'] = (_res, _args[:-1] + [c_int, c_float, P])
 
 
+class ReduceJob(ctypes.Structure):
+    _fields_ = [('slabs', P), ('num_slabs', c_int), ('slab_stride', c_long),
+                ('batch', c_int), ('in_batch_stride', c_long),
+                ('offset', c_long), ('n', c_long), ('dst', P),
+                ('out_batch_stride', c_long), ('replicate', c_int),
+                ('rep_stride', c_long)]
+
+
+def reduce_jobs(jobs):
+    return (ReduceJob * len(jobs))(*[ReduceJob(*j) for j in jobs])
+
 
 _lib = None
 
diff --git a/tensorflow-wavenet_amd/wavenet/fastgen.py b/tensorflow-wavenet_amd/wavenet/fastgen.py
--- a/tensorflow-wavenet_amd/wavenet/fastgen.py
+++ b/tensorflow-wavenet_amd/wavenet/fastgen.py
@@ -214,6 +214,7 @@
     ws = net._workspace(1, n0, False)
     for codes, gc, streams, lc in groups:
         ws.q.copy_(codes)
+        ws.from_audio = False
         lcond.fill(net, lc, ws)
         train_pass.run_pass(net, 'fwd', ws, net._gc_ids(gc, 1),
                             train_pass.step_path(net, ws, False))
diff --git a/tensorflow-wavenet_amd/wavenet/model.py b/tensorflow-wavenet_amd/wavenet/model.py
--- a/tensorflow-wavenet_amd/wavenet/model.py
+++ b/tensorflow-wavenet_amd/wavenet/model.py
@@ -565,7 +565,7 @@
                                    a.shape[1], 'loss')
         lc = lcond.check(self, local_condition_batch, local_condition_offset,
                          B, a.shape[1], 'loss')
-        return self._loss(mu_law_encode(a, self.Q), global_condition_batch,
+        return self._loss(None, global_condition_batch,
                           l2_regularization_strength, backward, a, lc, mask,
                           hist)
 
@@ -588,7 +588,7 @@
 
     def _loss(self, q, global_condition_batch, l2_regularization_strength,
               backward, audio, lc, mask=None, hist=None):
-        B, T = q.shape
+        B, T = audio.shape if q is None else q.shape
         N = B * T
         ws = self._workspace(B, T, backward)
         if backward and self._tail_work is not None:
@@ -598,16 +598,22 @@
                           'was never joined (no optimizer.minimize followed): '
                           'joined and dropped now')
             parallel.abandon_tail_allreduce(self)
-        ws.q.copy_(q.reshape(-1))
-        if self.scalar_input:
-            if audio is None:
-                raise ValueError('scalar_input needs the float audio')
+        path = train_pass.step_path(
+            self, ws, backward, l2=l2_regularization_strength is not None)
+        ws.from_audio = q is None and train_pass.uses_prologue(self, path)
+        if ws.from_audio:
             ws.audio.copy_(audio.reshape(-1))
+        else:
+            if q is None:
+                q = mu_law_encode(audio, self.Q)
+            ws.q.copy_(q.reshape(-1))
+            if self.scalar_input:
+                if audio is None:
+                    raise ValueError('scalar_input needs the float audio')
+                ws.audio.copy_(audio.reshape(-1))
         ids = self._gc_ids(global_condition_batch, B)
         st = _lib.stream()
         lcond.fill(self, lc, ws)
-        path = train_pass.step_path(
-            self, ws, backward, l2=l2_regularization_strength is not None)
         train_pass.run_pass(self, 'fwd', ws, ids, path)
         quirk = 1 if self.tf_xent_zero_label_quirk else 0
         if mask is None:
@@ -730,6 +736,7 @@
         lc = lcond.rows(self, local_condition, B, T, 'predict_proba')
         ws = self._workspace(B, T, False)
         ws.q.copy_(w.reshape(-1))
+        ws.from_audio = False
         if self.scalar_input:
             ws.audio.copy_(mu_law_decode(w, self.Q).reshape(-1))
         ids = self._gc_ids(global_condition, B)
diff --git a/tensorflow-wavenet_amd/wavenet/scoring.py b/tensorflow-wavenet_amd/wavenet/scoring.py
--- a/tensorflow-wavenet_amd/wavenet/scoring.py
+++ b/tensorflow-wavenet_amd/wavenet/scoring.py
@@ -14,6 +14,7 @@
     B, T = q.shape
     ws = net._workspace(B, T, False)
     ws.q.copy_(q.reshape(-1))
+    ws.from_audio = False
     if net.scalar_input:
         if audio is None:
             raise ValueError('scalar_input needs the float audio')
diff --git a/tensorflow-wavenet_amd/wavenet/train_pass.py b/tensorflow-wavenet_amd/wavenet/train_pass.py
--- a/tensorflow-wavenet_amd/wavenet/train_pass.py
+++ b/tensorflow-wavenet_amd/wavenet/train_pass.py
@@ -40,6 +40,10 @@
                     net.gemm_mode, ws.stack_variant)
 
 
+def uses_prologue(net, path):
+    return path.fwd.startswith('stack') and not net.scalar_input
+
+
 def early_allreduce(net):
     from . import parallel
     _lib.call_py(lambda: parallel.begin_tail_allreduce(net))
@@ -105,7 +109,7 @@
     if not net.use_launch_plans or (tag == 'bwd' and path.bwd == 'blocked'):
         return eager(net, ws, ids, path)
     key = (tag, path, ids is not None, _lib.stream(),
-           net.params.data_ptr(), net.grads.data_ptr())
+           net.params.data_ptr(), net.grads.data_ptr(), ws.from_audio)
     plan = ws.plans.get(key, 0)
     if plan == 0:
         ws.plans[key] = None
@@ -123,7 +127,10 @@
     B, T, N, L, S, Q = ws.B, ws.T, ws.N, net.L, net.S, net.Q
     P = net.params
     wc = net._seg(P, 'causal')
-    for cb in range(net.CB):
+    pro = uses_prologue(net, path)
+    if pro:
+        step_prologue(net, ws, path, st)
+    for cb in range(net.CB) if not pro else ():
         if net.scalar_input:
             _lib.call('wn_scalar_causal_fwd', _lib.ptr(ws.audio),
                       _lib.ptr(wc[cb * CH:]), net.CHn, _lib.ptr(ws.X[cb]),
@@ -159,8 +166,9 @@
     fuse_skip = path.fwd == 'stack_skip'
     bsum = None
     if net.use_biases and not fuse_skip:
-        _lib.call('wn_sum_rows', _lib.ptr(net._seg(P, 'skip_b')), L, S,
-                  _lib.ptr(ws.bsum), st)
+        if not pro:
+            _lib.call('wn_sum_rows', _lib.ptr(net._seg(P, 'skip_b')), L, S,
+                      _lib.ptr(ws.bsum), st)
         bsum = ws.bsum
     LP, C = L * net.CB, net.CHn
     b1 = net._seg(P, 'post1_b') if net.use_biases else None
@@ -183,12 +191,38 @@
          None, 0, _lib.ptr(ws.logits), Q, 0, 0, None, N, Q, S, 0)])
 
 
+def step_prologue(net, ws, path, st):
+    P, L, S, Q = net.params, net.L, net.S, net.Q
+    bwd = path.bwd is not None
+    thr = None
+    if ws.from_audio:
+        from .ops import mu_law_tables
+        thr = mu_law_tables(Q)[0]
+    ub = net.use_biases
+    _lib.call('wn_step_prologue', _lib.ptr(net._layer_block(P, 0)),
+              net.layer_stride, _lib.ptr(ws.wimg_f),
+              _lib.ptr(ws.wimg_b) if path.pack_both else None, L,
+              _lib.ptr(net._seg(P, 'post2_w')),
+              _lib.ptr(ws.w2t) if bwd else None,
+              _lib.ptr(net._seg(P, 'post1_w')),
+              _lib.ptr(ws.w1t) if bwd else None,
+              _lib.ptr(net._seg(P, 'skip_w')),
+              _lib.ptr(ws.wst) if bwd else None, S, Q,
+              _lib.ptr(net._seg(P, 'skip_b')) if ub else None,
+              _lib.ptr(ws.bsum) if ub else None,
+              _lib.ptr(ws.audio) if ws.from_audio else None, _lib.ptr(thr),
+              _lib.ptr(ws.q), _lib.ptr(net._seg(P, 'causal')),
+              _lib.ptr(ws.X[0]), ws.B, ws.T, st)
+
+
 def fwd_stack(net, ws, path, bias, bstride, st):
     B, T, N, L, S = ws.B, ws.T, ws.N, net.L, net.S
     P = net.params
-    _lib.call('wn_stack_pack', _lib.ptr(net._layer_block(P, 0)),
-              net.layer_stride, _lib.ptr(ws.wimg_f),
-              _lib.ptr(ws.wimg_b) if path.pack_both else None, L, st)
+    pro = uses_prologue(net, path)
+    if not pro:
+        _lib.call('wn_stack_pack', _lib.ptr(net._layer_block(P, 0)),
+                  net.layer_stride, _lib.ptr(ws.wimg_f),
+                  _lib.ptr(ws.wimg_b) if path.pack_both else None, L, st)
     save = path.save_ts != 0
     stack_args = (_lib.ptr(ws.X), _lib.ptr(ws.Z),
                   _lib.ptr(ws.SG) if save else None,
@@ -206,8 +240,9 @@
                 dtype=torch.float32, device=net.device)
         bsum_f = None
         if net.use_biases:
-            _lib.call('wn_sum_rows', _lib.ptr(net._seg(P, 'skip_b')), L,
-                      S, _lib.ptr(ws.bsum), st)
+            if not pro:
+                _lib.call('wn_sum_rows', _lib.ptr(net._seg(P, 'skip_b')), L,
+                          S, _lib.ptr(ws.bsum), st)
             bsum_f = ws.bsum
         _lib.call('wn_stack_skip_pack', _lib.ptr(net._seg(P, 'skip_w')),
                   L, _lib.ptr(ws.skimg), st)
@@ -249,12 +284,13 @@
     rp = net.residual_postproc
     dlog = ws.logits
     LP, C = L * net.CB, net.CHn
-    _lib.call('wn_transpose', _lib.ptr(net._seg(P, 'post2_w')), S, Q, Q,
-              _lib.ptr(ws.w2t), S, st)
-    _lib.call('wn_transpose', _lib.ptr(net._seg(P, 'post1_w')), S, S, S,
-              _lib.ptr(ws.w1t), S, st)
-    _lib.call('wn_transpose', _lib.ptr(net._seg(P, 'skip_w')), L * C, S,
-              S, _lib.ptr(ws.wst), L * C, st)
+    if not uses_prologue(net, path):
+        _lib.call('wn_transpose', _lib.ptr(net._seg(P, 'post2_w')), S, Q, Q,
+                  _lib.ptr(ws.w2t), S, st)
+        _lib.call('wn_transpose', _lib.ptr(net._seg(P, 'post1_w')), S, S, S,
+                  _lib.ptr(ws.w1t), S, st)
+        _lib.call('wn_transpose', _lib.ptr(net._seg(P, 'skip_w')), L * C, S,
+                  S, _lib.ptr(ws.wst), L * C, st)
     nn_dc1 = (_lib.ptr(dlog), Q, 0, 0, _lib.ptr(ws.w2t), S,
               None, _lib.ptr(ws.c1 if rp else ws.h2), S, None, 0,
               _lib.ptr(ws.dc1), S, 0, 0, _lib.ptr(ws.dh2) if rp else None,
@@ -439,30 +475,37 @@
     B, T, N, L, Q = ws.B, ws.T, ws.N, net.L, net.Q
     P, Gr = net.params, net.grads
     stack = path.bwd.startswith('stack')
+    jobs = []
     if path.bwd != 'layer_k' and ws.dsum is not None:
         tile_rows = ws.stack_rows if stack else 32
         tpc = (T + tile_rows - 1) // tile_rows
-        _lib.call('wn_reduce_slabs', _lib.ptr(ws.tilesum), tpc, 64, L * B,
-                  tpc * 64, 0, 64, _lib.ptr(ws.dsum), 64, 1, 0, st)
+        jobs.append((_lib.ptr(ws.tilesum), tpc, 64, L * B, tpc * 64, 0, 64,
+                     _lib.ptr(ws.dsum), 64, 1, 0))
     reg = ws.region['layers_stack' if stack else
                     'layers_2' if path.bwd == 'layer2' else 'layers_k']
     lo, _ = net.segments['layers']
-    _lib.call('wn_reduce_slabs', _lib.ptr(reg.buf), reg.count, reg.stride, L,
-              ws.lslabs.shape[1] * reg.stride, 0, reg.n, _lib.ptr(Gr[lo:]),
-              net.layer_stride, 1, 0, st)
+    jobs.append((_lib.ptr(reg.buf), reg.count, reg.stride, L,
+                 ws.lslabs.shape[1] * reg.stride, 0, reg.n,
+                 _lib.ptr(Gr[lo:]), net.layer_stride, 1, 0))
     gc_ = net._seg(Gr, 'causal')
+    if path.causal_wgrad == 'segsum':
+        reg = ws.region['causal_segsum']
+        _lib.call('wn_causal_wgrad', _lib.ptr(ws.q), _lib.ptr(dxin),
+                  _lib.ptr(reg.buf), reg.count, B, T, Q, st)
+        jobs.append((_lib.ptr(reg.buf), reg.count, reg.stride, 1, 0, 0,
+                     reg.n, _lib.ptr(gc_), 0, 1, 0))
+        _lib.call('wn_reduce_slabs_multi', _lib.reduce_jobs(jobs), len(jobs),
+                  st)
+        jobs = []
+    for j in jobs:
+        _lib.call('wn_reduce_slabs', *j, st)
     if path.causal_wgrad == 'scalar':
         reg = ws.region['causal_scalar']
         _lib.call('wn_scalar_causal_wgrad', _lib.ptr(ws.audio),
                   _lib.ptr(dxin), _lib.ptr(reg.buf), reg.count, B, T,
                   net.initial_filter_width, st)
         reduce_slabs(reg, _lib.ptr(gc_), st)
-    elif path.causal_wgrad == 'segsum':
-        reg = ws.region['causal_segsum']
-        _lib.call('wn_causal_wgrad', _lib.ptr(ws.q), _lib.ptr(dxin),
-                  _lib.ptr(reg.buf), reg.count, B, T, Q, st)
-        reduce_slabs(reg, _lib.ptr(gc_), st)
-    else:
+    elif path.causal_wgrad != 'segsum':
         K, reg = net.KW, ws.region['causal_onehot']
         for tap in range(K):
             shift = (K - 1 - tap) + (K - 1) // 2
diff --git a/tensorflow-wavenet_amd/wavenet/workspace.py b/tensorflow-wavenet_amd/wavenet/workspace.py
--- a/tensorflow-wavenet_amd/wavenet/workspace.py
+++ b/tensorflow-wavenet_amd/wavenet/workspace.py
@@ -45,7 +45,8 @@
         alloc('q', (N,), torch.int32)
         self.gc_ids = alloc('gc_ids', (B,), torch.int32) \
             if net.card is not None else None
-        self.audio = alloc('audio', (N,)) if net.scalar_input else None
+        alloc('audio', (N,))
+        self.from_audio = False
         alloc('X', (LP, N, CH))
         alloc('Z', (LP, N, CH))
         alloc('h1', (N, S))
```

New measurement: 13.56 million (median of 3 runs). Within noise of the previous version (+0.1%).
